# underdoc-wang/STC-GNN

Hardware: NVIDIA B200
Metric: train samples/s (fwd+bwd), SF-shape STC cell stack (higher is better)
Workload: dtype f32

## Files before the change

### stc_gnn_b200/csrc/stc_conv_tc.cu

```cuda
#include "stc_conv_common.cuh"
#include "stc_tc.cuh"

#include <stdlib.h>

namespace stc {

using namespace tc;

struct TcFwdPlan {
  int npt;
  int Dp;
  int KBL;
  int KB;
  int Ntot;
  int Npad;
  int nacc;
  int nmain;
  int tmem_cols;
  int ntiles;
  int x_bulk;
  int PS;
  uint32_t off_a, off_b, off_sh, off_sx, off_se, off_q, off_bias, off_bar, smem_bytes;
};

__device__ __forceinline__ void tc_issue_tile_loads(const ConvArgs& a, const TcFwdPlan& p, int tile, float* stage_h,
                                                    float* stage_x, uint64_t* bar) {
  const long long total_nodes = (long long)a.B * a.N;
  const long long g0 = (long long)tile * p.npt;
  const int nv = (int)min((long long)p.npt, total_nodes - g0);
  const long long R = total_nodes * a.C;
  const int CH = a.C * a.h, CD = a.C * a.Din;
  uint32_t bytes = (uint32_t)(a.Ks * nv * CH * 4);
  if (p.x_bulk) bytes += (uint32_t)(a.Ks * nv * CD * 4);
  mbar_arrive_expect_tx(bar, bytes);
  for (int k = 0; k < a.Ks; ++k) {
    const float* hsrc = (k == 0 ? a.h0 : a.yh + (long long)(k - 1) * R * a.h) + g0 * CH;
    bulk_g2s(stage_h + (size_t)k * 128 * a.h, hsrc, (uint32_t)(nv * CH * 4), bar);
    if (!p.x_bulk) continue;
    float* dst = stage_x + (size_t)k * 128 * a.Din;
    if (k > 0) {
      bulk_g2s(dst, a.yx + (long long)(k - 1) * R * a.Din + g0 * CD, (uint32_t)(nv * CD * 4), bar);
    } else {
      long long g = g0;
      int left = nv;
      while (left > 0) {
        const long long b = g / a.N;
        const int m = (int)(g - b * a.N);
        const int seg = min(left, a.N - m);
        bulk_g2s(dst, a.x0 + b * a.x0_bs + (long long)m * CD, (uint32_t)(seg * CD * 4), bar);
        dst += seg * CD;
        g += seg;
        left -= seg;
      }
    }
  }
}

__device__ __forceinline__ void tc_prefetch_tile(const ConvArgs& a, const TcFwdPlan& p, int tile) {
  const long long total_nodes = (long long)a.B * a.N;
  const long long g0 = (long long)tile * p.npt;
  const int nv = (int)min((long long)p.npt, total_nodes - g0);
  const long long R = total_nodes * a.C;
  const int CH = a.C * a.h, CD = a.C * a.Din;
  const uint32_t hb = (uint32_t)(nv * CH * 4), xb = (uint32_t)(nv * CD * 4);
  for (int k = 0; k < a.Ks; ++k) {
    l2_prefetch((k == 0 ? a.h0 : a.yh + (long long)(k - 1) * R * a.h) + g0 * CH, hb);
    if (!p.x_bulk) continue;
    if (k > 0) {
      l2_prefetch(a.yx + (long long)(k - 1) * R * a.Din + g0 * CD, xb);
    } else {
      long long g = g0;
      int left = nv;
      while (left > 0) {
        const long long b = g / a.N;
        const int m = (int)(g - b * a.N);
        const int seg = min(left, a.N - m);
        l2_prefetch(a.x0 + b * a.x0_bs + (long long)m * CD, (uint32_t)(seg * CD * 4));
        g += seg;
        left -= seg;
      }
    }
  }
  if (a.Hprev != a.h0) l2_prefetch(a.Hprev + g0 * CH, hb);
  if (a.phase != 0) l2_prefetch(a.u + g0 * CH, hb);
}

constexpr int TC_APM = 3;

__device__ __forceinline__ void tc_read_acc8(uint32_t tl, const TcFwdPlan& p, int c0, float (&v)[8]) {
  if (p.nmain == 1) {
    uint32_t t0[8], t1[8];
    tmem_ld8_async(tl + (uint32_t)(p.Npad + c0), t1);
    tmem_ld8_async(tl + (uint32_t)c0, t0);
    tmem_ld_wait();
    tmem_ld_pin8(t0); tmem_ld_pin8(t1);
#pragma unroll
    for (int i = 0; i < 8; ++i) v[i] = __uint_as_float(t1[i]) + __uint_as_float(t0[i]);
    return;
  }
  float t[8];
  tmem_ld8(tl + (uint32_t)(p.nmain * p.Npad + c0), v);
  for (int m = 0; m < p.nmain; ++m) {
    tmem_ld8(tl + (uint32_t)(m * p.Npad + c0), t);
#pragma unroll
    for (int i = 0; i < 8; ++i) v[i] += t[i];
  }
}

template <int NG>
__device__ __forceinline__ void tc_fwd_epilogue_fast(const ConvArgs& a, const TcFwdPlan& p, uint32_t tl, float* Pm,
                                                     const float* Qs, const float* bias_s, const float* stage_e,
                                                     int erow, int enode, int ecat, int half, bool valid,
                                                     long long gr) {
  const int h = a.h, C = a.C, Hout = a.Hout;
  const int cb = half * 8;
  uint32_t sm1[NG][8], mn1[NG][8];
#pragma unroll
  for (int g = 0; g < NG; ++g) {
    tmem_ld8_async(tl + (uint32_t)(p.Npad + Hout + 16 * g + cb), sm1[g]);
    tmem_ld8_async(tl + (uint32_t)(Hout + 16 * g + cb), mn1[g]);
  }
  tmem_ld_wait();
#pragma unroll
  for (int g = 0; g < NG; ++g) {
    tmem_ld_pin8(sm1[g]); tmem_ld_pin8(mn1[g]);
    float t[8];
#pragma unroll
    for (int i = 0; i < 8; ++i) t[i] = __uint_as_float(sm1[g][i]) + __uint_as_float(mn1[g][i]);
    float* pm = Pm + erow * p.PS + 16 * g + cb;
    *reinterpret_cast<float4*>(pm) = make_float4(t[0], t[1], t[2], t[3]);
    *reinterpret_cast<float4*>(pm + 4) = make_float4(t[4], t[5], t[6], t[7]);
    if (a.Psave && valid) {
      float* ps = a.Psave + gr * (long long)Hout + 16 * g + cb;
      *reinterpret_cast<float4*>(ps) = make_float4(t[0], t[1], t[2], t[3]);
      *reinterpret_cast<float4*>(ps + 4) = make_float4(t[4], t[5], t[6], t[7]);
    }
  }
  uint32_t sm0[NG][8], mn0[NG][8];
#pragma unroll
  for (int g = 0; g < NG; ++g) {
    tmem_ld8_async(tl + (uint32_t)(p.Npad + 16 * g + cb), sm0[g]);
    tmem_ld8_async(tl + (uint32_t)(16 * g + cb), mn0[g]);
  }
  __syncthreads();
  tmem_ld_wait();
  float v[NG][8];
#pragma unroll
  for (int g = 0; g < NG; ++g) {
    tmem_ld_pin8(sm0[g]); tmem_ld_pin8(mn0[g]);
#pragma unroll
    for (int i = 0; i < 8; ++i) v[g][i] = __uint_as_float(sm0[g][i]) + __uint_as_float(mn0[g][i]);
  }
  {
    const float* pp = Pm + (enode * C) * p.PS + cb;
#pragma unroll 5
    for (int cp = 0; cp < C; ++cp) {
      const float w = Qs[cp * C + ecat];
#pragma unroll
      for (int g = 0; g < NG; ++g) {
        const float4 x0 = *reinterpret_cast<const float4*>(pp + cp * p.PS + 16 * g);
        const float4 x1 = *reinterpret_cast<const float4*>(pp + cp * p.PS + 16 * g + 4);
        v[g][0] = fmaf(w, x0.x, v[g][0]); v[g][1] = fmaf(w, x0.y, v[g][1]);
        v[g][2] = fmaf(w, x0.z, v[g][2]); v[g][3] = fmaf(w, x0.w, v[g][3]);
        v[g][4] = fmaf(w, x1.x, v[g][4]); v[g][5] = fmaf(w, x1.y, v[g][5]);
        v[g][6] = fmaf(w, x1.z, v[g][6]); v[g][7] = fmaf(w, x1.w, v[g][7]);
      }
    }
  }
  if (!valid) return;
#pragma unroll
  for (int g = 0; g < NG; ++g) {
    const float4 b0 = *reinterpret_cast<const float4*>(bias_s + 16 * g + cb);
    const float4 b1 = *reinterpret_cast<const float4*>(bias_s + 16 * g + cb + 4);
    v[g][0] += b0.x; v[g][1] += b0.y; v[g][2] += b0.z; v[g][3] += b0.w;
    v[g][4] += b1.x; v[g][5] += b1.y; v[g][6] += b1.z; v[g][7] += b1.w;
    if (a.act == STC_ACT_RELU) {
#pragma unroll
      for (int i = 0; i < 8; ++i) v[g][i] = fmaxf(v[g][i], 0.f);
    }
  }
  if (a.phase == 0) {
#pragma unroll
    for (int g = 0; g < NG; ++g) {
#pragma unroll
      for (int i = 0; i < 8; ++i) v[g][i] = sigmoidf_fast(v[g][i]);
      const int col = 16 * g + cb;
      if (col < h) {
        float* dst = a.u + gr * h + col;
        *reinterpret_cast<float4*>(dst) = make_float4(v[g][0], v[g][1], v[g][2], v[g][3]);
        *reinterpret_cast<float4*>(dst + 4) = make_float4(v[g][4], v[g][5], v[g][6], v[g][7]);
      } else {
        const int ch = col - h;
        const float4 h0 = *reinterpret_cast<const float4*>(stage_e + erow * h + ch);
        const float4 h1 = *reinterpret_cast<const float4*>(stage_e + erow * h + ch + 4);
        float* dr = a.r + gr * h + ch;
        *reinterpret_cast<float4*>(dr) = make_float4(v[g][0], v[g][1], v[g][2], v[g][3]);
        *reinterpret_cast<float4*>(dr + 4) = make_float4(v[g][4], v[g][5], v[g][6], v[g][7]);
        float* drh = a.rH + gr * h + ch;
        *reinterpret_cast<float4*>(drh) = make_float4(v[g][0] * h0.x, v[g][1] * h0.y, v[g][2] * h0.z, v[g][3] * h0.w);
        *reinterpret_cast<float4*>(drh + 4) = make_float4(v[g][4] * h1.x, v[g][5] * h1.y, v[g][6] * h1.z, v[g][7] * h1.w);
      }
    }
  } else {
#pragma unroll
    for (int g = 0; g < NG; ++g) {
      const int col = 16 * g + cb;
      const long long o = gr * h + col;
      float cc[8], hn[8];
      const float4 u0 = *reinterpret_cast<const float4*>(stage_e + 128 * h + erow * h + col);
      const float4 u1 = *reinterpret_cast<const float4*>(stage_e + 128 * h + erow * h + col + 4);
      const float4 p0 = *reinterpret_cast<const float4*>(stage_e + erow * h + col);
      const float4 p1 = *reinterpret_cast<const float4*>(stage_e + erow * h + col + 4);
      const float uu[8] = {u0.x, u0.y, u0.z, u0.w, u1.x, u1.y, u1.z, u1.w};
      const float hp[8] = {p0.x, p0.y, p0.z, p0.w, p1.x, p1.y, p1.z, p1.w};
#pragma unroll
      for (int i = 0; i < 8; ++i) {
        cc[i] = tanhf_fast(v[g][i]);
        hn[i] = fmaf(uu[i], cc[i] - hp[i], hp[i]);
      }
      *reinterpret_cast<float4*>(a.c + o) = make_float4(cc[0], cc[1], cc[2], cc[3]);
      *reinterpret_cast<float4*>(a.c + o + 4) = make_float4(cc[4], cc[5], cc[6], cc[7]);
      *reinterpret_cast<float4*>(a.Hnew + o) = make_float4(hn[0], hn[1], hn[2], hn[3]);
      *reinterpret_cast<float4*>(a.Hnew + o + 4) = make_float4(hn[4], hn[5], hn[6], hn[7]);
    }
  }
}

template <int NG>
__global__ void __launch_bounds__(CV_THREADS, 2)
tc_conv_fwd_kernel(const ConvArgs a, const TcFwdPlan p) {
  extern __shared__ __align__(1024) uint8_t smem[];
  if ((smem_u32(smem) & 1023u) != 0u) __trap();
  const int tid = threadIdx.x, warp = tid >> 5, lane = tid & 31;
  const int C = a.C, L = a.Din + a.h, h = a.h, Din = a.Din, Hout = a.Hout;
  const uint32_t atomA = 128 * ATOM_ROW_BYTES;
  const uint32_t atomB = (uint32_t)p.Npad * ATOM_ROW_BYTES;
  uint8_t* A_hi = smem + p.off_a;
  uint8_t* A_lo = A_hi + atomA;
  float* Pm = reinterpret_cast<float*>(A_hi);
  uint8_t* B_hi = smem + p.off_b;
  uint8_t* B_lo = B_hi + (size_t)p.nacc * atomB;
  float* stage_h = reinterpret_cast<float*>(smem + p.off_sh);
  float* stage_x = reinterpret_cast<float*>(smem + p.off_sx);
  float* Qs = reinterpret_cast<float*>(smem + p.off_q);
  float* bias_s = reinterpret_cast<float*>(smem + p.off_bias);
  float* stage_e = reinterpret_cast<float*>(smem + p.off_se);
  uint64_t* mma_bar = reinterpret_cast<uint64_t*>(smem + p.off_bar);
  uint64_t* load_bar = mma_bar + 1;
  uint64_t* epi_bar = mma_bar + 2;
  uint32_t* tmem_slot = reinterpret_cast<uint32_t*>(mma_bar + 3);

  if (tid == 0) {
    mbar_init(mma_bar, 1);
    mbar_init(load_bar, 1);
    mbar_init(epi_bar, 1);
    mbar_fence_init();
  }
  if (warp == 0) tmem_alloc(tmem_slot, (uint32_t)p.tmem_cols);
  for (int i = tid; i < (a.Kc - 1) * C * C; i += CV_THREADS) Qs[i] = a.Q[C * C + i];
  for (int i = tid; i < Hout; i += CV_THREADS) bias_s[i] = a.bias ? a.bias[i] : 0.f;
  for (int i = tid; i < a.Ks * 128 * h; i += CV_THREADS) stage_h[i] = 0.f;
  for (int i = tid; i < a.Ks * 128 * Din; i += CV_THREADS) stage_x[i] = 0.f;
  for (int k = 0; k < a.Ks; ++k)
    for (int j = 0; j < p.KB; ++j) {
      uint8_t* bh = B_hi + (size_t)(k * p.KB + j) * atomB;
      uint8_t* bl = B_lo + (size_t)(k * p.KB + j) * atomB;
      for (int it = tid; it < p.Npad * 8; it += CV_THREADS) {
        const int n = it >> 3, qq = it & 7;
        const int c = n / Hout, o = n - c * Hout;
        float v[4];
#pragma unroll
        for (int i = 0; i < 4; ++i) {
          const int kb = j * ATOM_K + qq * 4 + i;
          const int l = kb < h ? Din + kb : (kb - h < Din ? kb - h : -1);
          v[i] = (n < p.Ntot && l >= 0) ? a.W[((size_t)(k * a.Kc + c) * L + l) * Hout + o] : 0.f;
        }
        store_split4(bh, bl, atom_chunk_offset(n, qq), make_float4(v[0], v[1], v[2], v[3]));
      }
    }
  fence_async_smem();
  fence_before_sync();
  __syncthreads();
  fence_after_sync();
  const int warp_u = uniform_warp_index();
  const uint32_t tmem_base = uniform_u32(*tmem_slot);
  const uint32_t idesc = make_idesc_tf32(128, p.Npad);
  const uint32_t d_small = tmem_base + (uint32_t)(p.nmain * p.Npad);
  const long long total_nodes = (long long)a.B * a.N;
  const long long R = total_nodes * C;
  const uint64_t dA_hi = make_smem_desc_sw128(smem_u32(A_hi)), dA_lo = make_smem_desc_sw128(smem_u32(A_lo));
  const uint64_t dB_hi = make_smem_desc_sw128(smem_u32(B_hi)), dB_lo = make_smem_desc_sw128(smem_u32(B_lo));

  const int q = tid & 7, r0 = tid >> 3;
  uint32_t aoff[4];
#pragma unroll
  for (int i = 0; i < 4; ++i) aoff[i] = atom_chunk_offset(r0 + 32 * i, q);
  const int lane_base = (warp & 3) * 32, half = warp >> 2;
  const int erow = lane_base + lane;
  const int enode = erow / C, ecat = erow - enode * C;
  const uint32_t tl = tmem_base + ((uint32_t)lane_base << 16);

  uint32_t mma_phase = 0, load_phase = 0, epi_phase = 0;
  bool mma_pending = false;
  const bool tracing = a.trace != nullptr && blockIdx.x == 0 && tid == 0;
  int trace_it = 0;
  if (warp_u == 1 && elect_one_sync() && (int)blockIdx.x < p.ntiles) tc_issue_tile_loads(a, p, blockIdx.x, stage_h, stage_x, load_bar);

  for (int tile = blockIdx.x; tile < p.ntiles; tile += gridDim.x) {
    const long long g0 = (long long)tile * p.npt;
    const int nodes_valid = (int)min((long long)p.npt, total_nodes - g0);
    const int rows_valid = nodes_valid * C;
    STC_TRACE(0);
    if (warp_u == 1 && elect_one_sync()) {
      const uint32_t eb = (uint32_t)(rows_valid * h * 4);
      mbar_arrive_expect_tx(epi_bar, a.phase == 0 ? eb : 2 * eb);
      bulk_g2s(stage_e, a.Hprev + g0 * C * h, eb, epi_bar);
      if (a.phase != 0) bulk_g2s(stage_e + 128 * h, a.u + g0 * C * h, eb, epi_bar);
      if ((a.opt & OPT_L2_PREFETCH) && tile + (int)gridDim.x < p.ntiles) tc_prefetch_tile(a, p, tile + gridDim.x);
    }
    mbar_wait(load_bar, load_phase);
    load_phase ^= 1u;
    if (!p.x_bulk) {
      for (int k = 0; k < a.Ks; ++k) {
        float* dst = stage_x + (size_t)k * 128 * Din;
        const int per_node = C * Din;
        for (int idx = tid; idx < nodes_valid * per_node; idx += CV_THREADS) {
          const int node = idx / per_node, rem = idx - node * per_node;
          const long long g = g0 + node;
          const float* src;
          if (k == 0) {
            const long long b = g / a.N;
            src = a.x0 + b * a.x0_bs + (g - b * a.N) * per_node;
          } else {
            src = a.yx + (long long)(k - 1) * R * Din + g * per_node;
          }
          dst[idx] = src[rem];
        }
      }
      __syncthreads();
    }
    STC_TRACE(1);
    bool acc_small = false;
    int ai = 0;
    for (int k = 0; k < a.Ks; ++k) {
      const float* sh = stage_h + (size_t)k * 128 * h;
      const float* sx = stage_x + (size_t)k * 128 * Din;
      for (int j = 0; j < p.KB; ++j, ++ai) {
        const int kb = j * ATOM_K + q * 4;
        const bool from_h = kb < h;
        float4 vv[4];
        if (from_h || (p.x_bulk && kb - h < Din)) {
          const float* bp = from_h ? sh + kb : sx + (kb - h);
          const int st = from_h ? h : Din;
#pragma unroll
          for (int i = 0; i < 4; ++i) vv[i] = *reinterpret_cast<const float4*>(bp + (r0 + 32 * i) * st);
        } else {
          const int xi = kb - h;
#pragma unroll
          for (int i = 0; i < 4; ++i) {
            float e[4] = {0.f, 0.f, 0.f, 0.f};
            const float* sp = sx + (r0 + 32 * i) * Din + xi;
#pragma unroll
            for (int t = 0; t < 4; ++t)
              if (xi + t < Din) e[t] = sp[t];
            vv[i] = make_float4(e[0], e[1], e[2], e[3]);
          }
        }
        float4 vh[4], vl[4];
#pragma unroll
        for (int i = 0; i < 4; ++i) {
          split_tf32(vv[i].x, vh[i].x, vl[i].x); split_tf32(vv[i].y, vh[i].y, vl[i].y);
          split_tf32(vv[i].z, vh[i].z, vl[i].z); split_tf32(vv[i].w, vh[i].w, vl[i].w);
        }
        if (mma_pending) {
          mbar_wait(mma_bar, mma_phase);
          mma_phase ^= 1u;
          mma_pending = false;
          if (ai == p.nacc - 1) STC_TRACE(3);
        }
#pragma unroll
        for (int i = 0; i < 4; ++i) {
          *reinterpret_cast<float4*>(A_hi + aoff[i]) = vh[i];
          *reinterpret_cast<float4*>(A_lo + aoff[i]) = vl[i];
        }
        if (ai == 0) STC_TRACE(12);
        fence_async_smem();
        if (ai == 0) STC_TRACE(13);
        __syncthreads();
        if (ai == 0) STC_TRACE(2);
        if (warp_u == 1 && ai == p.nacc - 1 && tile + (int)gridDim.x < p.ntiles && elect_one_sync())
          tc_issue_tile_loads(a, p, tile + gridDim.x, stage_h, stage_x, load_bar);
        if (warp_u == 0 && elect_one_sync()) {
          fence_after_sync();
          const int kleft = p.KBL - j * ATOM_K;
          const int ksteps = kleft >= ATOM_K ? 4 : (kleft + 7) / 8;
          const uint64_t bo = (uint64_t)(((uint32_t)ai * atomB) >> 4);
          const uint32_t d_main = tmem_base + (uint32_t)((ai / TC_APM) * p.Npad);
          uint32_t acc_main = (ai % TC_APM) != 0 ? 1u : 0u;
#pragma unroll 4
          for (int ks = 0; ks < ksteps; ++ks) {
            const uint64_t ko = (uint64_t)(ks * 2);
            mma_tf32(d_small, dA_lo + ko, dB_hi + bo + ko, idesc, acc_small ? 1u : 0u);
            mma_tf32(d_small, dA_hi + ko, dB_lo + bo + ko, idesc, 1u);
            mma_tf32(d_main, dA_hi + ko, dB_hi + bo + ko, idesc, acc_main);
            acc_main = 1u;
            acc_small = true;
          }
          if (ai == 0) STC_TRACE(8);
          if (ai == p.nacc - 1) STC_TRACE(10);
          mma_commit(mma_bar);
          if (ai == 0) STC_TRACE(9);
          if (ai == p.nacc - 1) STC_TRACE(11);
        }
        acc_small = true;
        mma_pending = true;
      }
    }
    STC_TRACE(4);
    mbar_wait(mma_bar, mma_phase);
    mma_phase ^= 1u;
    mma_pending = false;
    fence_after_sync();
    STC_TRACE(5);
    mbar_wait(epi_bar, epi_phase);
    epi_phase ^= 1u;
    STC_TRACE(6);
    const bool valid = erow < rows_valid;
    const long long gr = g0 * C + erow;
    if constexpr (NG != 0) {
      tc_fwd_epilogue_fast<NG>(a, p, tl, Pm, Qs, bias_s, stage_e, erow, enode, ecat, half, valid, gr);
    } else {
      for (int c0 = half * 8; c0 < Hout; c0 += 16) {
        float v[8];
        tc_read_acc8(tl, p, c0, v);
        for (int c = 1; c < a.Kc; ++c) {
          float t[8];
          tc_read_acc8(tl, p, c * Hout + c0, t);
          __syncthreads();
          *reinterpret_cast<float4*>(Pm + erow * p.PS + c0) = make_float4(t[0], t[1], t[2], t[3]);
          *reinterpret_cast<float4*>(Pm + erow * p.PS + c0 + 4) = make_float4(t[4], t[5], t[6], t[7]);
          if (a.Psave && valid) {
            float4* ps = reinterpret_cast<float4*>(a.Psave + gr * (long long)((a.Kc - 1) * Hout) + (c - 1) * Hout + c0);
            ps[0] = make_float4(t[0], t[1], t[2], t[3]);
            ps[1] = make_float4(t[4], t[5], t[6], t[7]);
          }
          __syncthreads();
          const float* Qc = Qs + (size_t)(c - 1) * C * C;
          const float* pp = Pm + (enode * C) * p.PS + c0;
          for (int cp = 0; cp < C; ++cp) {
            const float w = Qc[cp * C + ecat];
            const float4 x0 = *reinterpret_cast<const float4*>(pp + cp * p.PS);
            const float4 x1 = *reinterpret_cast<const float4*>(pp + cp * p.PS + 4);
            v[0] = fmaf(w, x0.x, v[0]); v[1] = fmaf(w, x0.y, v[1]); v[2] = fmaf(w, x0.z, v[2]); v[3] = fmaf(w, x0.w, v[3]);
            v[4] = fmaf(w, x1.x, v[4]); v[5] = fmaf(w, x1.y, v[5]); v[6] = fmaf(w, x1.z, v[6]); v[7] = fmaf(w, x1.w, v[7]);
          }
        }
        if (!valid) continue;
#pragma unroll
        for (int i = 0; i < 8; ++i) {
          float pre = v[i] + bias_s[c0 + i];
          if (a.act == STC_ACT_RELU) pre = fmaxf(pre, 0.f);
          v[i] = pre;
        }
        if (a.phase == 0) {
#pragma unroll
          for (int i = 0; i < 8; ++i) v[i] = sigmoidf_fast(v[i]);
          if (c0 < h) {
            float4* dst = reinterpret_cast<float4*>(a.u + gr * h + c0);
            dst[0] = make_float4(v[0], v[1], v[2], v[3]);
            dst[1] = make_float4(v[4], v[5], v[6], v[7]);
          } else {
            const long long o = gr * h + (c0 - h);
            const float4 h0 = *reinterpret_cast<const float4*>(stage_e + erow * h + (c0 - h));
            const float4 h1 = *reinterpret_cast<const float4*>(stage_e + erow * h + (c0 - h) + 4);
            float4* dr = reinterpret_cast<float4*>(a.r + o);
            dr[0] = make_float4(v[0], v[1], v[2], v[3]);
            dr[1] = make_float4(v[4], v[5], v[6], v[7]);
            float4* drh = reinterpret_cast<float4*>(a.rH + o);
            drh[0] = make_float4(v[0] * h0.x, v[1] * h0.y, v[2] * h0.z, v[3] * h0.w);
            drh[1] = make_float4(v[4] * h1.x, v[5] * h1.y, v[6] * h1.z, v[7] * h1.w);
          }
        } else {
          const long long o = gr * h + c0;
          float uu[8], hp[8], cc[8], hn[8];
          *reinterpret_cast<float4*>(uu) = *reinterpret_cast<const float4*>(stage_e + 128 * h + erow * h + c0);
          *reinterpret_cast<float4*>(uu + 4) = *reinterpret_cast<const float4*>(stage_e + 128 * h + erow * h + c0 + 4);
          *reinterpret_cast<float4*>(hp) = *reinterpret_cast<const float4*>(stage_e + erow * h + c0);
          *reinterpret_cast<float4*>(hp + 4) = *reinterpret_cast<const float4*>(stage_e + erow * h + c0 + 4);
#pragma unroll
          for (int i = 0; i < 8; ++i) {
            cc[i] = tanhf_fast(v[i]);
            hn[i] = fmaf(uu[i], cc[i] - hp[i], hp[i]);
          }
          float4* dc = reinterpret_cast<float4*>(a.c + o);
          dc[0] = make_float4(cc[0], cc[1], cc[2], cc[3]);
          dc[1] = make_float4(cc[4], cc[5], cc[6], cc[7]);
          float4* dh = reinterpret_cast<float4*>(a.Hnew + o);
          dh[0] = make_float4(hn[0], hn[1], hn[2], hn[3]);
          dh[1] = make_float4(hn[4], hn[5], hn[6], hn[7]);
        }
      }
    }
    STC_TRACE(7);
    ++trace_it;
    fence_before_sync();
    fence_async_smem();
    __syncthreads();
  }
  __syncthreads();
  if (warp == 0) tmem_dealloc(tmem_base, (uint32_t)p.tmem_cols);
}

template <int NG>
__device__ __forceinline__ void tc_fwd_epilogue_regs(const ConvArgs& a, const TcFwdPlan& p, uint32_t tl, float* Pm,
                                                     const float* Qs, const float* bias_s, const float4 (&hp)[2],
                                                     const float4 (&uu)[2], int erow, int enode, int ecat, int half,
                                                     bool valid, long long gr) {
  const int h = a.h, C = a.C, Hout = a.Hout;
  const int cb = half * 8;
  uint32_t sm1[NG][8], mn1[NG][8];
#pragma unroll
  for (int g = 0; g < NG; ++g) {
    tmem_ld8_async(tl + (uint32_t)(p.Npad + Hout + 16 * g + cb), sm1[g]);
    tmem_ld8_async(tl + (uint32_t)(Hout + 16 * g + cb), mn1[g]);
  }
  tmem_ld_wait();
#pragma unroll
  for (int g = 0; g < NG; ++g) {
    tmem_ld_pin8(sm1[g]); tmem_ld_pin8(mn1[g]);
    float t[8];
#pragma unroll
    for (int i = 0; i < 8; ++i) t[i] = __uint_as_float(sm1[g][i]) + __uint_as_float(mn1[g][i]);
    float* pm = Pm + erow * p.PS + 16 * g + cb;
    *reinterpret_cast<float4*>(pm) = make_float4(t[0], t[1], t[2], t[3]);
    *reinterpret_cast<float4*>(pm + 4) = make_float4(t[4], t[5], t[6], t[7]);
    if (a.Psave && valid) {
      float* ps = a.Psave + gr * (long long)Hout + 16 * g + cb;
      *reinterpret_cast<float4*>(ps) = make_float4(t[0], t[1], t[2], t[3]);
      *reinterpret_cast<float4*>(ps + 4) = make_float4(t[4], t[5], t[6], t[7]);
    }
  }
  uint32_t sm0[NG][8], mn0[NG][8];
#pragma unroll
  for (int g = 0; g < NG; ++g) {
    tmem_ld8_async(tl + (uint32_t)(p.Npad + 16 * g + cb), sm0[g]);
    tmem_ld8_async(tl + (uint32_t)(16 * g + cb), mn0[g]);
  }
  __syncthreads();
  tmem_ld_wait();
  float v[NG][8];
#pragma unroll
  for (int g = 0; g < NG; ++g) {
    tmem_ld_pin8(sm0[g]); tmem_ld_pin8(mn0[g]);
#pragma unroll
    for (int i = 0; i < 8; ++i) v[g][i] = __uint_as_float(sm0[g][i]) + __uint_as_float(mn0[g][i]);
  }
  {
    const float* pp = Pm + (enode * C) * p.PS + cb;
#pragma unroll 5
    for (int cp = 0; cp < C; ++cp) {
      const float w = Qs[cp * C + ecat];
#pragma unroll
      for (int g = 0; g < NG; ++g) {
        const float4 x0 = *reinterpret_cast<const float4*>(pp + cp * p.PS + 16 * g);
        const float4 x1 = *reinterpret_cast<const float4*>(pp + cp * p.PS + 16 * g + 4);
        v[g][0] = fmaf(w, x0.x, v[g][0]); v[g][1] = fmaf(w, x0.y, v[g][1]);
        v[g][2] = fmaf(w, x0.z, v[g][2]); v[g][3] = fmaf(w, x0.w, v[g][3]);
        v[g][4] = fmaf(w, x1.x, v[g][4]); v[g][5] = fmaf(w, x1.y, v[g][5]);
        v[g][6] = fmaf(w, x1.z, v[g][6]); v[g][7] = fmaf(w, x1.w, v[g][7]);
      }
    }
  }
  if (!valid) return;
#pragma unroll
  for (int g = 0; g < NG; ++g) {
    const float4 b0 = *reinterpret_cast<const float4*>(bias_s + 16 * g + cb);
    const float4 b1 = *reinterpret_cast<const float4*>(bias_s + 16 * g + cb + 4);
    v[g][0] += b0.x; v[g][1] += b0.y; v[g][2] += b0.z; v[g][3] += b0.w;
    v[g][4] += b1.x; v[g][5] += b1.y; v[g][6] += b1.z; v[g][7] += b1.w;
    if (a.act == STC_ACT_RELU) {
#pragma unroll
      for (int i = 0; i < 8; ++i) v[g][i] = fmaxf(v[g][i], 0.f);
    }
  }
  const float hpv[8] = {hp[0].x, hp[0].y, hp[0].z, hp[0].w, hp[1].x, hp[1].y, hp[1].z, hp[1].w};
  if (a.phase == 0) {
#pragma unroll
    for (int g = 0; g < NG; ++g) {
#pragma unroll
      for (int i = 0; i < 8; ++i) v[g][i] = sigmoidf_fast(v[g][i]);
      const int col = 16 * g + cb;
      if (col < h) {
        float* dst = a.u + gr * h + col;
        *reinterpret_cast<float4*>(dst) = make_float4(v[g][0], v[g][1], v[g][2], v[g][3]);
        *reinterpret_cast<float4*>(dst + 4) = make_float4(v[g][4], v[g][5], v[g][6], v[g][7]);
      } else {
        const int ch = col - h;
        float* dr = a.r + gr * h + ch;
        *reinterpret_cast<float4*>(dr) = make_float4(v[g][0], v[g][1], v[g][2], v[g][3]);
        *reinterpret_cast<float4*>(dr + 4) = make_float4(v[g][4], v[g][5], v[g][6], v[g][7]);
        float* drh = a.rH + gr * h + ch;
        *reinterpret_cast<float4*>(drh) = make_float4(v[g][0] * hpv[0], v[g][1] * hpv[1], v[g][2] * hpv[2], v[g][3] * hpv[3]);
        *reinterpret_cast<float4*>(drh + 4) = make_float4(v[g][4] * hpv[4], v[g][5] * hpv[5], v[g][6] * hpv[6], v[g][7] * hpv[7]);
      }
    }
  } else {
    const float uuv[8] = {uu[0].x, uu[0].y, uu[0].z, uu[0].w, uu[1].x, uu[1].y, uu[1].z, uu[1].w};
    const long long o = gr * h + cb;
    float cc[8], hn[8];
#pragma unroll
    for (int i = 0; i < 8; ++i) {
      cc[i] = tanhf_fast(v[0][i]);
      hn[i] = fmaf(uuv[i], cc[i] - hpv[i], hpv[i]);
    }
    *reinterpret_cast<float4*>(a.c + o) = make_float4(cc[0], cc[1], cc[2], cc[3]);
    *reinterpret_cast<float4*>(a.c + o + 4) = make_float4(cc[4], cc[5], cc[6], cc[7]);
    *reinterpret_cast<float4*>(a.Hnew + o) = make_float4(hn[0], hn[1], hn[2], hn[3]);
    *reinterpret_cast<float4*>(a.Hnew + o + 4) = make_float4(hn[4], hn[5], hn[6], hn[7]);
  }
}

template <int NG>
__global__ void __launch_bounds__(CV_THREADS, 2)
tc_conv_fwd_at_kernel(const ConvArgs a, const TcFwdPlan p) {
  extern __shared__ __align__(1024) uint8_t smem[];
  if ((smem_u32(smem) & 1023u) != 0u) __trap();
  const int tid = threadIdx.x, warp = tid >> 5, lane = tid & 31;
  const int C = a.C, L = a.Din + a.h, Din = a.Din, Hout = a.Hout;
  constexpr int h = 16;
  const uint32_t atomB = (uint32_t)p.Npad * ATOM_ROW_BYTES;
  float* Pm = reinterpret_cast<float*>(smem + p.off_a);
  uint8_t* B_hi = smem + p.off_b;
  uint8_t* B_lo = B_hi + atomB;
  float* Qs = reinterpret_cast<float*>(smem + p.off_q);
  float* bias_s = reinterpret_cast<float*>(smem + p.off_bias);
  uint64_t* mma_bar = reinterpret_cast<uint64_t*>(smem + p.off_bar);
  uint32_t* tmem_slot = reinterpret_cast<uint32_t*>(mma_bar + 1);

  if (tid == 0) {
    mbar_init(mma_bar, 1);
    mbar_fence_init();
  }
  if (warp == 0) tmem_alloc(tmem_slot, (uint32_t)p.tmem_cols);
  for (int i = tid; i < C * C; i += CV_THREADS) Qs[i] = a.Q[C * C + i];
  for (int i = tid; i < Hout; i += CV_THREADS) bias_s[i] = a.bias ? a.bias[i] : 0.f;
  for (int k = 0; k < 2; ++k) {
    uint8_t* bh = B_hi + (size_t)k * 2 * atomB;
    uint8_t* bl = B_lo + (size_t)k * 2 * atomB;
    for (int it = tid; it < p.Npad * 8; it += CV_THREADS) {
      const int n = it >> 3, qq = it & 7;
      const int c = n / Hout, o = n - c * Hout;
      float v[4];
#pragma unroll
      for (int i = 0; i < 4; ++i) {
        const int kb = qq * 4 + i;
        const int l = kb < h ? Din + kb : (kb - h < Din ? kb - h : -1);
        v[i] = (n < p.Ntot && l >= 0) ? a.W[((size_t)(k * 2 + c) * L + l) * Hout + o] : 0.f;
      }
      store_split4(bh, bl, atom_chunk_offset(n, qq), make_float4(v[0], v[1], v[2], v[3]));
    }
  }
  fence_async_smem();
  fence_before_sync();
  __syncthreads();
  fence_after_sync();
  const int warp_u = uniform_warp_index();
  const uint32_t tmem_base = uniform_u32(*tmem_slot);
  const uint32_t idesc = make_idesc_tf32(128, p.Npad), idesc2 = make_idesc_tf32(128, 2 * p.Npad);
  const uint32_t d_main = tmem_base, d_small = tmem_base + (uint32_t)p.Npad;
  const uint32_t colA = (uint32_t)(2 * p.Npad);
  const uint64_t dB_hi = make_smem_desc_sw128(smem_u32(B_hi));
  const int ksteps = p.KBL >> 3;
  const long long total_nodes = (long long)a.B * a.N;
  const long long R = total_nodes * C;

  const int sp = warp & 3, half = warp >> 2;
  const int erow = sp * 32 + lane;
  const int enode = erow / C, ecat = erow - enode * C;
  const uint32_t tl = tmem_base + ((uint32_t)(sp * 32) << 16);
  const uint32_t tA = tl + colA + (uint32_t)(half * 32);
  const bool xvec = p.x_bulk != 0;
  uint32_t mma_phase = 0;
  const bool tracing = a.trace != nullptr && blockIdx.x == 0 && tid == 0;
  int trace_it = 0;
  for (int tile = blockIdx.x; tile < p.ntiles; tile += gridDim.x) {
    const long long g0 = (long long)tile * p.npt;
    const int nodes_valid = (int)min((long long)p.npt, total_nodes - g0);
    const int rows_valid = nodes_valid * C;
    const bool valid = erow < rows_valid;
    const long long gr = g0 * C + erow;
    STC_TRACE(0);
    if ((a.opt & OPT_L2_PREFETCH) && warp_u == 1 && tile + (int)gridDim.x < p.ntiles && elect_one_sync())
      tc_prefetch_tile(a, p, tile + gridDim.x);
    float4 xv[8];
#pragma unroll
    for (int i = 0; i < 8; ++i) xv[i] = make_float4(0.f, 0.f, 0.f, 0.f);
    if (valid) {
      const float* hs = (half == 0 ? a.h0 : a.yh) + gr * h;
#pragma unroll
      for (int i = 0; i < 4; ++i) xv[i] = *reinterpret_cast<const float4*>(hs + 4 * i);
      const float* xs;
      if (half == 0) {
        const long long g = g0 + enode;
        const long long b = g / a.N;
        xs = a.x0 + b * a.x0_bs + ((g - b * a.N) * C + ecat) * Din;
      } else {
        xs = a.yx + gr * Din;
      }
      if (xvec) {
#pragma unroll
        for (int i = 0; i < 4; ++i)
          if (4 * i < Din) xv[4 + i] = *reinterpret_cast<const float4*>(xs + 4 * i);
      } else {
        float e[16];
#pragma unroll
        for (int i = 0; i < 16; ++i) e[i] = i < Din ? xs[i] : 0.f;
#pragma unroll
        for (int i = 0; i < 4; ++i) xv[4 + i] = make_float4(e[4 * i], e[4 * i + 1], e[4 * i + 2], e[4 * i + 3]);
      }
    }
    STC_TRACE(1);
#pragma unroll
    for (int i = 0; i < 4; ++i) {
      float hi[8], lo[8];
      split_tf32(xv[2 * i].x, hi[0], lo[0]); split_tf32(xv[2 * i].y, hi[1], lo[1]);
      split_tf32(xv[2 * i].z, hi[2], lo[2]); split_tf32(xv[2 * i].w, hi[3], lo[3]);
      split_tf32(xv[2 * i + 1].x, hi[4], lo[4]); split_tf32(xv[2 * i + 1].y, hi[5], lo[5]);
      split_tf32(xv[2 * i + 1].z, hi[6], lo[6]); split_tf32(xv[2 * i + 1].w, hi[7], lo[7]);
      tmem_st8(tA + (uint32_t)(8 * i), hi);
      tmem_st8(tA + 64u + (uint32_t)(8 * i), lo);
    }
    tmem_st_wait();
    STC_TRACE(12);
    fence_before_sync();
    STC_TRACE(13);
    __syncthreads();
    STC_TRACE(2);
    STC_TRACE(3);
    if (warp_u == 0 && elect_one_sync()) {
      fence_after_sync();
      uint32_t acc = 0u;
#pragma unroll
      for (int ai = 0; ai < 2; ++ai) {
        const uint64_t bo = (uint64_t)(((uint32_t)ai * 2u * atomB) >> 4);
        for (int ks = 0; ks < ksteps; ++ks) {
          const uint64_t ko = (uint64_t)(ks * 2);
          const uint32_t ah = tmem_base + colA + (uint32_t)(ai * 32 + ks * 8), al = ah + 64u;
          mma_tf32_atmem(d_main, ah, dB_hi + bo + ko, idesc2, acc);
          mma_tf32_atmem(d_small, al, dB_hi + bo + ko, idesc, 1u);
          acc = 1u;
        }
      }
      STC_TRACE(8);
      STC_TRACE(10);
      mma_commit(mma_bar);
      STC_TRACE(9);
      STC_TRACE(11);
    }
    float4 hp[2], uu[2];
    hp[0] = hp[1] = uu[0] = uu[1] = make_float4(0.f, 0.f, 0.f, 0.f);
    if (valid) {
      const float* hsrc = a.Hprev + gr * h + half * 8;
      hp[0] = *reinterpret_cast<const float4*>(hsrc);
      hp[1] = *reinterpret_cast<const float4*>(hsrc + 4);
      if (a.phase != 0) {
        const float* usrc = a.u + gr * h + half * 8;
        uu[0] = *reinterpret_cast<const float4*>(usrc);
        uu[1] = *reinterpret_cast<const float4*>(usrc + 4);
      }
    }
    STC_TRACE(4);
    mbar_wait(mma_bar, mma_phase);
    mma_phase ^= 1u;
    fence_after_sync();
    STC_TRACE(5);
    STC_TRACE(6);
    tc_fwd_epilogue_regs<NG>(a, p, tl, Pm, Qs, bias_s, hp, uu, erow, enode, ecat, half, valid, gr);
    STC_TRACE(7);
    ++trace_it;
    fence_before_sync();
    __syncthreads();
  }
  __syncthreads();
  if (warp == 0) tmem_dealloc(tmem_base, (uint32_t)p.tmem_cols);
}

static bool tc_disabled() {
  static int cached = -1;
  if (cached < 0) {
    const char* e = getenv("STC_DISABLE_TC");
    cached = (e && e[0] && e[0] != '0') ? 1 : 0;
  }
  return cached == 1;
}

static bool aligned16p(const void* p) { return (reinterpret_cast<uintptr_t>(p) & 15) == 0; }

bool conv_tc_eligible(const ConvArgs& a) {
  if (tc_disabled()) return false;
  if (a.h % 8 != 0 || a.Hout % 16 != 0 || a.C > 128) return false;
  const int Dp = (a.Din + 7) & ~7, KBL = a.h + Dp, KB = (KBL + ATOM_K - 1) / ATOM_K;
  const int Nf = (a.Kc * a.Hout + 15) & ~15;
  if (Nf > 256 || (a.Ks * KB + 1) * Nf > 512) return false;
  if ((size_t)128 * (a.Hout + 4) * sizeof(float) > 2 * 128 * ATOM_ROW_BYTES) return false;
  const size_t fwd_smem = 2 * 128 * ATOM_ROW_BYTES + 2 * (size_t)a.Ks * KB * Nf * ATOM_ROW_BYTES +
                          (size_t)a.Ks * 128 * (a.h + a.Din) * sizeof(float) + (size_t)2 * 128 * a.h * sizeof(float) +
                          (size_t)a.Kc * a.C * a.C * sizeof(float) + 64;
  if (fwd_smem > 200 * 1024) return false;
  const int Nb = (a.Ks * KBL + 15) & ~15, KA = (a.Kc * a.Hout + ATOM_K - 1) / ATOM_K;
  if (Nb > 256 || (KA + 1) * Nb > 512) return false;
  const size_t dx_smem = 2 * 128 * ATOM_ROW_BYTES + 2 * (size_t)KA * Nb * ATOM_ROW_BYTES +
                         (size_t)128 * (a.Hout + 4 + a.h + (a.Kc - 1) * a.Hout) * sizeof(float) +
                         (size_t)2 * a.Kc * a.C * a.C * sizeof(float) + 256;
  if (dx_smem > 200 * 1024) return false;
  return true;
}

int try_launch_conv_fwd_tc(const ConvArgs& a, cudaStream_t st, bool* handled) {
  *handled = false;
  if (!conv_tc_eligible(a)) return STC_OK;
  const int L = a.Din + a.h, P = a.Ks * a.Kc;
  if (!aligned16p(a.u) || !aligned16p(a.Hprev) || !aligned16p(a.r) || !aligned16p(a.rH) || !aligned16p(a.c) ||
      !aligned16p(a.Hnew) || !aligned16p(a.h0) || !aligned16p(a.yh) || !aligned16p(a.Psave)) {
    set_error("tcgen05 path needs 16-byte aligned state / workspace tensors");
    return STC_ERR_BAD_ARG;
  }
  auto declined = [&](const char* why) {
    set_error("tcgen05 forward declined an eligible shape (%s): N=%d C=%d Din=%d h=%d Ks=%d Kc=%d Hout=%d", why, a.N, a.C,
              a.Din, a.h, a.Ks, a.Kc, a.Hout);
    return STC_ERR_UNSUPPORTED;
  };
  TcFwdPlan p;
  p.npt = 128 / a.C;
  p.Dp = (a.Din + 7) & ~7;
  p.KBL = a.h + p.Dp;
  p.KB = (p.KBL + ATOM_K - 1) / ATOM_K;
  p.Ntot = a.Kc * a.Hout;
  p.Npad = (p.Ntot + 15) & ~15;
  if (p.Npad > 256) return declined("N tile");
  p.nacc = a.Ks * p.KB;
  p.nmain = (p.nacc + TC_APM - 1) / TC_APM;
  p.tmem_cols = 32;
  while (p.tmem_cols < (p.nmain + 1) * p.Npad) p.tmem_cols *= 2;
  if (p.tmem_cols > 512) return declined("tensor memory columns");
  p.PS = a.Hout + 4;
  if ((size_t)128 * p.PS * sizeof(float) > 2 * 128 * ATOM_ROW_BYTES) return declined("exchange buffer");
  p.x_bulk = (a.Din % 4 == 0) && (a.x0_bs % 4 == 0) && aligned16p(a.x0) && aligned16p(a.yx);
  const long long total_nodes = (long long)a.B * a.N;
  p.ntiles = ceil_div(total_nodes, p.npt);
  const size_t atomB = (size_t)p.Npad * ATOM_ROW_BYTES;
  size_t o = 0;
  p.off_a = (uint32_t)o; o += 2 * 128 * ATOM_ROW_BYTES;
  p.off_b = (uint32_t)o; o += 2 * (size_t)p.nacc * atomB;
  p.off_sh = (uint32_t)o; o += (size_t)a.Ks * 128 * a.h * sizeof(float);
  p.off_sx = (uint32_t)o; o += round_up((size_t)a.Ks * 128 * a.Din * sizeof(float), 16);
  p.off_se = (uint32_t)o; o += (size_t)2 * 128 * a.h * sizeof(float);
  p.off_q = (uint32_t)o; o += (size_t)(a.Kc > 1 ? a.Kc - 1 : 0) * a.C * a.C * sizeof(float);
  o = round_up(o, 16);
  p.off_bias = (uint32_t)o; o += (size_t)a.Hout * sizeof(float);
  o = round_up(o, 16);
  p.off_bar = (uint32_t)o; o += 48;
  p.smem_bytes = (uint32_t)o;
  const bool smem_over = p.smem_bytes > 200 * 1024;
  int ng = 0;
  if (a.Kc == 2 && p.nmain == 1 && (a.Hout == 16 || a.Hout == 32) && !(a.opt & OPT_GENERIC_EPILOGUE)) ng = a.Hout / 16;
  auto kern = ng == 2 ? tc_conv_fwd_kernel<2> : (ng == 1 ? tc_conv_fwd_kernel<1> : tc_conv_fwd_kernel<0>);
  const bool at = ng != 0 && a.Ks == 2 && a.h == 16 && p.KB == 1 && !(a.opt & OPT_SMEM_A);
  if (at) {
    kern = ng == 2 ? tc_conv_fwd_at_kernel<2> : tc_conv_fwd_at_kernel<1>;
    size_t q = 0;
    p.off_a = (uint32_t)q; q += round_up((size_t)128 * p.PS * sizeof(float), 1024);
    p.off_b = (uint32_t)q; q += 2 * (size_t)2 * atomB;
    p.off_q = (uint32_t)q; q += round_up((size_t)a.C * a.C * sizeof(float), 16);
    p.off_bias = (uint32_t)q; q += round_up((size_t)a.Hout * sizeof(float), 16);
    p.off_bar = (uint32_t)q; q += 32;
    p.smem_bytes = (uint32_t)q;
    p.tmem_cols = 256;
  }
  if (!at && smem_over) return declined("shared memory");
  STC_TRY(set_smem(kern, p.smem_bytes));
  int ctas_per_sm = (int)((228 * 1024) / (p.smem_bytes + 1024));
  if (ctas_per_sm < 1) ctas_per_sm = 1;
  if (ctas_per_sm > 2) ctas_per_sm = 2;
  if (ctas_per_sm * p.tmem_cols > 512) ctas_per_sm = 512 / p.tmem_cols;
  int grid = device_sm_count() * ctas_per_sm;
  if (grid > p.ntiles) grid = p.ntiles;
  const double R = (double)total_nodes * a.C;
  ScopedKernelTimer _t(KK_TC_CONV_FWD, st,
                       4.0 * R * (a.Ks * L + (a.phase == 0 ? 3 * a.h : 4 * a.h)) + 4.0 * P * L * a.Hout);
  kern<<<grid, CV_THREADS, p.smem_bytes, st>>>(a, p);
  STC_LAUNCH_OK("tc_conv_fwd_kernel");
  *handled = true;
  return STC_OK;
}

__global__ void __launch_bounds__(CV_THREADS, 1)
tf32x3_gemm_kernel(const float* __restrict__ A, const float* __restrict__ Bm, float* __restrict__ D, int M, int N,
                   int K, int Npad, int tmem_cols, int mode, int nmain, int small) {
  extern __shared__ __align__(1024) uint8_t smem[];
  if ((smem_u32(smem) & 1023u) != 0u) __trap();
  const int tid = threadIdx.x, warp = tid >> 5, lane = tid & 31;
  const uint32_t atomA = 128 * ATOM_ROW_BYTES, atomB = (uint32_t)Npad * ATOM_ROW_BYTES;
  uint8_t* A_hi = smem;
  uint8_t* A_lo = A_hi + atomA;
  uint8_t* B_hi = A_lo + atomA;
  uint8_t* B_lo = B_hi + atomB;
  uint64_t* bar = reinterpret_cast<uint64_t*>(B_lo + atomB);
  uint32_t* tmem_slot = reinterpret_cast<uint32_t*>(bar + 1);
  if (tid == 0) {
    mbar_init(bar, 1);
    mbar_fence_init();
  }
  if (warp == 0) tmem_alloc(tmem_slot, (uint32_t)tmem_cols);
  fence_before_sync();
  __syncthreads();
  fence_after_sync();
  const uint32_t tmem_base = *tmem_slot;
  const uint32_t idesc = make_idesc_tf32(128, Npad);
  const int m0 = blockIdx.x * 128;
  uint32_t phase = 0;
  bool acc_main[16], acc_small = false;
  for (int i = 0; i < 16; ++i) acc_main[i] = false;
  const int natoms = (K + ATOM_K - 1) / ATOM_K;
  for (int j = 0; j < natoms; ++j) {
    if (j > 0) {
      mbar_wait(bar, phase);
      phase ^= 1u;
    }
    for (int it = tid; it < 128 * 8; it += CV_THREADS) {
      const int row = it >> 3, q = it & 7;
      float v[4], hi[4], lo[4];
#pragma unroll
      for (int i = 0; i < 4; ++i) {
        const int k = j * ATOM_K + q * 4 + i;
        v[i] = (m0 + row < M && k < K) ? A[(size_t)(m0 + row) * K + k] : 0.f;
        if (mode & 1) split_tf32_trunc(v[i], hi[i], lo[i]); else split_tf32(v[i], hi[i], lo[i]);
      }
      const uint32_t off = atom_chunk_offset(row, q);
      *reinterpret_cast<float4*>(A_hi + off) = make_float4(hi[0], hi[1], hi[2], hi[3]);
      *reinterpret_cast<float4*>(A_lo + off) = make_float4(lo[0], lo[1], lo[2], lo[3]);
    }
    for (int it = tid; it < Npad * 8; it += CV_THREADS) {
      const int n = it >> 3, q = it & 7;
      float v[4], hi[4], lo[4];
#pragma unroll
      for (int i = 0; i < 4; ++i) {
        const int k = j * ATOM_K + q * 4 + i;
        v[i] = (n < N && k < K) ? Bm[(size_t)k * N + n] : 0.f;
        if (mode & 1) split_tf32_trunc(v[i], hi[i], lo[i]); else split_tf32(v[i], hi[i], lo[i]);
      }
      const uint32_t off = atom_chunk_offset(n, q);
      *reinterpret_cast<float4*>(B_hi + off) = make_float4(hi[0], hi[1], hi[2], hi[3]);
      *reinterpret_cast<float4*>(B_lo + off) = make_float4(lo[0], lo[1], lo[2], lo[3]);
    }
    fence_async_smem();
    __syncthreads();
    if (tid == 0) {
      fence_after_sync();
      const int kleft = K - j * ATOM_K;
      const int ksteps = kleft >= ATOM_K ? 4 : (kleft + 7) / 8;
      const int mi = j % nmain;
      const uint32_t d_main = tmem_base + (uint32_t)(mi * Npad);
      if (small) {
        const uint32_t d_small = tmem_base + (uint32_t)(nmain * Npad);
        mma_atom_3x_split(d_main, d_small, smem_u32(A_hi), smem_u32(A_lo), smem_u32(B_hi), smem_u32(B_lo), ksteps, idesc,
                          acc_main[mi], acc_small);
      } else {
        mma_atom_3x(d_main, smem_u32(A_hi), smem_u32(A_lo), smem_u32(B_hi), smem_u32(B_lo), ksteps, idesc, acc_main[mi]);
      }
      mma_commit(bar);
    }
  }
  mbar_wait(bar, phase);
  fence_after_sync();
  {
    const int lane_base = (warp & 3) * 32, half = warp >> 2;
    const int row = m0 + lane_base + lane;
    const int nchunks = Npad / 8;
    const int nbuf = (natoms < nmain ? natoms : nmain);
    for (int ch = half; ch < nchunks; ch += 2) {
      float acc[8], v[8];
      if (small) {
        tmem_ld8(tmem_base + ((uint32_t)lane_base << 16) + (uint32_t)(nmain * Npad + ch * 8), acc);
      } else {
        for (int i = 0; i < 8; ++i) acc[i] = 0.f;
      }
      for (int b = 0; b < nbuf; ++b) {
        tmem_ld8(tmem_base + ((uint32_t)lane_base << 16) + (uint32_t)(b * Npad + ch * 8), v);
        for (int i = 0; i < 8; ++i) acc[i] += v[i];
      }
      if (row < M)
        for (int i = 0; i < 8; ++i)
          if (ch * 8 + i < N) D[(size_t)row * N + ch * 8 + i] = acc[i];
    }
  }
  fence_before_sync();
  __syncthreads();
  if (warp == 0) tmem_dealloc(tmem_base, (uint32_t)tmem_cols);
}

struct MnLayout {
  int variant;
  uint32_t colblk;
  uint32_t kgroup;
  __device__ __forceinline__ uint32_t off(int k, int ch) const {
    if (variant == 2) return (uint32_t)(k >> 3) * kgroup + (uint32_t)ch * 128u + (uint32_t)(k & 7) * 16u;
    return (uint32_t)(ch >> 3) * colblk + mn32_chunk_offset(k, ch & 7);
  }
  __device__ __forceinline__ uint64_t desc(uint32_t base, int ks) const {
    if (variant == 2) {
      uint64_t d = 0;
      d |= (uint64_t)(((base + ks * kgroup) >> 4) & 0x3FFF);
      d |= (uint64_t)((kgroup >> 4) & 0x3FFF) << 16;
      d |= (uint64_t)((128u >> 4) & 0x3FFF) << 32;
      d |= (uint64_t)1 << 46;
      return d;
    }
    const uint32_t a = base + ks * 2 * MN32_GROUP_BYTES;
    return variant == 0 ? make_smem_desc_mn32(a, colblk, MN32_GROUP_BYTES) : make_smem_desc_mn32(a, MN32_GROUP_BYTES, colblk);
  }
};

__global__ void __launch_bounds__(CV_THREADS, 1)
tf32x3_gemm_mn_kernel(const float* __restrict__ A, const float* __restrict__ Bm, float* __restrict__ D, int M, int N,
                      int K, int Npad, int tmem_cols, int variant) {
  extern __shared__ __align__(1024) uint8_t smem[];
  if ((smem_u32(smem) & 1023u) != 0u) __trap();
  const int tid = threadIdx.x, warp = tid >> 5, lane = tid & 31;
  const int ncolB = (Npad + 31) / 32;
  const uint32_t colblk = 32 * ATOM_ROW_BYTES;
  const MnLayout la{variant, colblk, 32u * 128u};
  const MnLayout lb{variant, colblk, (uint32_t)(ncolB * 8) * 128u};
  uint8_t* A_hi = smem;
  uint8_t* A_lo = A_hi + 4 * colblk;
  uint8_t* B_hi = A_lo + 4 * colblk;
  uint8_t* B_lo = B_hi + ncolB * colblk;
  uint64_t* bar = reinterpret_cast<uint64_t*>(B_lo + ncolB * colblk);
  uint32_t* tmem_slot = reinterpret_cast<uint32_t*>(bar + 1);
  if (tid == 0) {
    mbar_init(bar, 1);
    mbar_fence_init();
  }
  if (warp == 0) tmem_alloc(tmem_slot, (uint32_t)tmem_cols);
  fence_before_sync();
  __syncthreads();
  fence_after_sync();
  const uint32_t tmem_base = *tmem_slot;
  const uint32_t idesc = make_idesc_tf32_mn(128, Npad);
  const int m0 = blockIdx.x * 128;
  uint32_t phase = 0;
  const int nchunksK = (K + 31) / 32;
  bool acc_main = false, acc_small = false;
  for (int j = 0; j < nchunksK; ++j) {
    if (j > 0) {
      mbar_wait(bar, phase);
      phase ^= 1u;
    }
    for (int it = tid; it < 32 * 32; it += CV_THREADS) {
      const int k = it >> 5, ch = it & 31;
      float v[4];
#pragma unroll
      for (int i = 0; i < 4; ++i) {
        const int m = ch * 4 + i, kk = j * 32 + k;
        v[i] = (m0 + m < M && kk < K) ? A[(size_t)(m0 + m) * K + kk] : 0.f;
      }
      store_split4(A_hi, A_lo, la.off(k, ch), make_float4(v[0], v[1], v[2], v[3]));
    }
    for (int it = tid; it < 32 * ncolB * 8; it += CV_THREADS) {
      const int k = it / (ncolB * 8), ch = it - k * (ncolB * 8);
      float v[4];
#pragma unroll
      for (int i = 0; i < 4; ++i) {
        const int n = ch * 4 + i, kk = j * 32 + k;
        v[i] = (n < N && kk < K) ? Bm[(size_t)kk * N + n] : 0.f;
      }
      store_split4(B_hi, B_lo, lb.off(k, ch), make_float4(v[0], v[1], v[2], v[3]));
    }
    fence_async_smem();
    __syncthreads();
    if (tid == 0) {
      fence_after_sync();
      const int kleft = K - j * 32;
      const int ksteps = kleft >= 32 ? 4 : (kleft + 7) / 8;
      for (int ks = 0; ks < ksteps; ++ks) {
        const uint64_t ah = la.desc(smem_u32(A_hi), ks), al = la.desc(smem_u32(A_lo), ks);
        const uint64_t bh = lb.desc(smem_u32(B_hi), ks), bl = lb.desc(smem_u32(B_lo), ks);
        mma_tf32(tmem_base + (uint32_t)Npad, al, bh, idesc, acc_small ? 1u : 0u);
        mma_tf32(tmem_base + (uint32_t)Npad, ah, bl, idesc, 1u);
        mma_tf32(tmem_base, ah, bh, idesc, acc_main ? 1u : 0u);
        acc_main = acc_small = true;
      }
      mma_commit(bar);
    }
  }
  mbar_wait(bar, phase);
  fence_after_sync();
  {
    const int lane_base = (warp & 3) * 32, half = warp >> 2;
    const int row = m0 + lane_base + lane;
    for (int ch = half; ch < Npad / 8; ch += 2) {
      float v[8], t[8];
      tmem_ld8(tmem_base + ((uint32_t)lane_base << 16) + (uint32_t)(Npad + ch * 8), v);
      tmem_ld8(tmem_base + ((uint32_t)lane_base << 16) + (uint32_t)(ch * 8), t);
      if (row < M)
        for (int i = 0; i < 8; ++i)
          if (ch * 8 + i < N) D[(size_t)row * N + ch * 8 + i] = v[i] + t[i];
    }
  }
  fence_before_sync();
  __syncthreads();
  if (warp == 0) tmem_dealloc(tmem_base, (uint32_t)tmem_cols);
}

int launch_tf32x3_gemm(const float* A, const float* Bm, float* D, int M, int N, int K, cudaStream_t st) {
  if (M <= 0 || N <= 0 || K <= 0 || N > 256) {
    set_error("tf32x3 gemm self-test: need M,K > 0 and 0 < N <= 256");
    return STC_ERR_BAD_ARG;
  }
  int mode = 0, nmain = 1, small = 0;
  if (const char* e = getenv("STC_TC_TEST_MODE")) mode = atoi(e);
  if (const char* e = getenv("STC_TC_TEST_NMAIN")) nmain = atoi(e);
  if (const char* e = getenv("STC_TC_TEST_SMALL")) small = atoi(e);
  const int Npad = (N + 15) & ~15;
  if (mode & 2) {
    int cols = 32;
    while (cols < 2 * Npad) cols *= 2;
    const size_t smem_mn = (size_t)(8 + 2 * ((Npad + 31) / 32)) * 32 * ATOM_ROW_BYTES + 64;
    STC_TRY(set_smem(tf32x3_gemm_mn_kernel, smem_mn));
    ScopedKernelTimer _t(KK_TC_GEMM_TEST, st, 4.0 * ((double)M * K + (double)K * N + (double)M * N));
    int variant = 0;
    if (const char* e = getenv("STC_TC_MN_VARIANT")) variant = atoi(e);
    tf32x3_gemm_mn_kernel<<<ceil_div(M, 128), CV_THREADS, smem_mn, st>>>(A, Bm, D, M, N, K, Npad, cols, variant);
    STC_LAUNCH_OK("tf32x3_gemm_mn_kernel");
    return STC_OK;
  }
  if (nmain < 1) nmain = 1;
  if (nmain > 15) nmain = 15;
  while ((nmain + (small ? 1 : 0)) * Npad > 512 && nmain > 1) --nmain;
  int tmem_cols = 32;
  while (tmem_cols < (nmain + (small ? 1 : 0)) * Npad) tmem_cols *= 2;
  const size_t smem = 2 * 128 * ATOM_ROW_BYTES + 2 * (size_t)Npad * ATOM_ROW_BYTES + 64;
  STC_TRY(set_smem(tf32x3_gemm_kernel, smem));
  ScopedKernelTimer _t(KK_TC_GEMM_TEST, st, 4.0 * ((double)M * K + (double)K * N + (double)M * N));
  tf32x3_gemm_kernel<<<ceil_div(M, 128), CV_THREADS, smem, st>>>(A, Bm, D, M, N, K, Npad, tmem_cols, mode, nmain, small);
  STC_LAUNCH_OK("tf32x3_gemm_kernel");
  return STC_OK;
}

}
```

### stc_gnn_b200/csrc/stc_conv_tc_bwd.cu

```cuda
#include "stc_conv_common.cuh"
#include "stc_tc.cuh"

namespace stc {

using namespace tc;

constexpr int DX_APM = 3;

struct TcDxPlan {
  int npt, Dp, KBL;
  int N1;
  int Npad;
  int Kdd;
  int KA;
  int nmain;
  int tmem_cols, ntiles;
  int DP;
  int PW;
  int x_vec;
  uint32_t off_a, off_b, off_ds, off_dh, off_ps, off_q, off_acc, off_bar, smem_bytes;
};

struct DxIn {
  float4 dhn, uu, cc, hp, rr, drh;
};
__device__ __forceinline__ void dx_load(const ConvArgs& a, long long o, DxIn& in) {
  in.dhn = *reinterpret_cast<const float4*>(a.dHn + o);
  in.uu = *reinterpret_cast<const float4*>(a.u + o);
  in.cc = *reinterpret_cast<const float4*>(a.c + o);
  if (a.phase == 0) {
    in.hp = *reinterpret_cast<const float4*>(a.Hprev + o);
    in.rr = *reinterpret_cast<const float4*>(a.r + o);
    in.drh = *reinterpret_cast<const float4*>(a.drH + o);
  }
}
__device__ __forceinline__ void dx_adjoint(const ConvArgs& a, const DxIn& in, float4& g0v, float4& g1v, float4& dir) {
  const float4 dhn = in.dhn, uu = in.uu, cc = in.cc;
  if (a.phase == 1) {
    g0v = make_float4(dhn.x * uu.x * (1.f - cc.x * cc.x), dhn.y * uu.y * (1.f - cc.y * cc.y),
                      dhn.z * uu.z * (1.f - cc.z * cc.z), dhn.w * uu.w * (1.f - cc.w * cc.w));
    if (a.act == STC_ACT_RELU) {
      if (!(cc.x > 0.f)) g0v.x = 0.f;
      if (!(cc.y > 0.f)) g0v.y = 0.f;
      if (!(cc.z > 0.f)) g0v.z = 0.f;
      if (!(cc.w > 0.f)) g0v.w = 0.f;
    }
  } else {
    const float4 hp = in.hp, rr = in.rr, drh = in.drh;
    g0v = make_float4(dhn.x * (cc.x - hp.x) * uu.x * (1.f - uu.x), dhn.y * (cc.y - hp.y) * uu.y * (1.f - uu.y),
                      dhn.z * (cc.z - hp.z) * uu.z * (1.f - uu.z), dhn.w * (cc.w - hp.w) * uu.w * (1.f - uu.w));
    g1v = make_float4(drh.x * hp.x * rr.x * (1.f - rr.x), drh.y * hp.y * rr.y * (1.f - rr.y),
                      drh.z * hp.z * rr.z * (1.f - rr.z), drh.w * hp.w * rr.w * (1.f - rr.w));
    if (a.act == STC_ACT_RELU) {
      if (!(uu.x > 0.5f)) g0v.x = 0.f;
      if (!(uu.y > 0.5f)) g0v.y = 0.f;
      if (!(uu.z > 0.5f)) g0v.z = 0.f;
      if (!(uu.w > 0.5f)) g0v.w = 0.f;
      if (!(rr.x > 0.5f)) g1v.x = 0.f;
      if (!(rr.y > 0.5f)) g1v.y = 0.f;
      if (!(rr.z > 0.5f)) g1v.z = 0.f;
      if (!(rr.w > 0.5f)) g1v.w = 0.f;
    }
    dir = make_float4(dhn.x * (1.f - uu.x) + drh.x * rr.x, dhn.y * (1.f - uu.y) + drh.y * rr.y,
                      dhn.z * (1.f - uu.z) + drh.z * rr.z, dhn.w * (1.f - uu.w) + drh.w * rr.w);
  }
}

__device__ __forceinline__ void dx_prefetch_tile(const ConvArgs& a, const TcDxPlan& p, int tile, bool want_dQ) {
  const long long total_nodes = (long long)a.B * a.N;
  const long long g0 = (long long)tile * p.npt;
  const int nv = (int)min((long long)p.npt, total_nodes - g0);
  const long long row0 = g0 * a.C;
  const uint32_t hb = (uint32_t)(nv * a.C * a.h * 4);
  l2_prefetch(a.dHn + row0 * a.h, hb);
  l2_prefetch(a.u + row0 * a.h, hb);
  l2_prefetch(a.c + row0 * a.h, hb);
  if (a.phase == 0) {
    l2_prefetch(a.Hprev + row0 * a.h, hb);
    l2_prefetch(a.r + row0 * a.h, hb);
    l2_prefetch(a.drH + row0 * a.h, hb);
  }
  if (want_dQ) l2_prefetch(a.Psave + row0 * p.PW, (uint32_t)(nv * a.C * p.PW * 4));
  if (a.accum_x && p.x_vec) {
    const uint32_t xb = (uint32_t)(nv * a.C * a.Din * 4);
    const long long R = total_nodes * a.C;
    if (a.dYx0) l2_prefetch(a.dYx0 + row0 * a.Din, xb);
    if (a.dYx)
      for (int k = 1; k < a.Ks; ++k) l2_prefetch(a.dYx + (size_t)(k - 1) * R * a.Din + row0 * a.Din, xb);
  }
}

template <bool FAST, bool AT>
__global__ void __launch_bounds__(CV_THREADS, 2)
tc_conv_bwd_dx_kernel(const ConvArgs a, const TcDxPlan p) {
  extern __shared__ __align__(1024) uint8_t smem[];
  if ((smem_u32(smem) & 1023u) != 0u) __trap();
  const int tid = threadIdx.x, warp = tid >> 5, lane = tid & 31;
  const int C = a.C, L = a.Din + a.h, h = a.h, Din = a.Din, Hout = a.Hout, DP = p.DP;
  const bool want_dQ = a.dQ != nullptr && a.Kc > 1;
  const uint32_t atomA = 128 * ATOM_ROW_BYTES;
  const uint32_t atomB = (uint32_t)p.Npad * ATOM_ROW_BYTES;
  uint8_t* A_hi = smem + p.off_a;
  uint8_t* A_lo = A_hi + atomA;
  uint8_t* B_hi = smem + p.off_b;
  uint8_t* B_lo = B_hi + (AT ? (size_t)atomB : (size_t)p.KA * atomB);
  const size_t bstride = AT ? 2 * (size_t)atomB : (size_t)atomB;
  float* Dsm = reinterpret_cast<float*>(smem + p.off_ds);
  float* Dh = reinterpret_cast<float*>(smem + p.off_dh);
  float* Psm = reinterpret_cast<float*>(smem + p.off_ps);
  float* Qs = reinterpret_cast<float*>(smem + p.off_q);
  float* dQacc = reinterpret_cast<float*>(smem + p.off_acc);
  uint64_t* mma_bar = reinterpret_cast<uint64_t*>(smem + p.off_bar);
  uint64_t* load_bar = mma_bar + 1;
  uint32_t* tmem_slot = reinterpret_cast<uint32_t*>(mma_bar + 2);

  if (tid == 0) {
    mbar_init(mma_bar, 1);
    mbar_init(load_bar, 1);
    mbar_fence_init();
  }
  if (warp == 0) tmem_alloc(tmem_slot, (uint32_t)p.tmem_cols);
  for (int i = tid; i < (a.Kc - 1) * C * C; i += CV_THREADS) {
    Qs[i] = a.Q[C * C + i];
    dQacc[i] = 0.f;
  }
  for (int ja = 0; ja < p.KA; ++ja) {
    uint8_t* bh = B_hi + (size_t)ja * bstride;
    uint8_t* bl = B_lo + (size_t)ja * bstride;
    for (int it = tid; it < p.Npad * 8; it += CV_THREADS) {
      const int n = it >> 3, qq = it & 7;
      const int k = n / p.KBL, kb = n - k * p.KBL;
      const int l = kb < h ? Din + kb : (kb - h < Din ? kb - h : -1);
      float v[4];
#pragma unroll
      for (int i = 0; i < 4; ++i) {
        const int kk = ja * ATOM_K + qq * 4 + i;
        const int c = kk / Hout, o = kk - c * Hout;
        v[i] = (n < p.N1 && l >= 0 && kk < p.Kdd) ? a.W[((size_t)(k * a.Kc + c) * L + l) * Hout + o] : 0.f;
      }
      store_split4(bh, bl, atom_chunk_offset(n, qq), make_float4(v[0], v[1], v[2], v[3]));
    }
  }
  fence_async_smem();
  fence_before_sync();
  __syncthreads();
  fence_after_sync();
  const int warp_u = uniform_warp_index();
  const uint32_t tmem_base = uniform_u32(*tmem_slot);
  const uint32_t idesc = make_idesc_tf32(128, p.Npad), idesc2 = make_idesc_tf32(128, 2 * p.Npad);
  const uint32_t d_small = tmem_base + (uint32_t)(p.nmain * p.Npad);
  const uint64_t dA_hi = make_smem_desc_sw128(smem_u32(A_hi)), dA_lo = make_smem_desc_sw128(smem_u32(A_lo));
  const uint64_t dB_hi = make_smem_desc_sw128(smem_u32(B_hi)), dB_lo = make_smem_desc_sw128(smem_u32(B_lo));
  const long long total_nodes = (long long)a.B * a.N;
  const long long R = total_nodes * C;

  const int q = tid & 7, r0 = tid >> 3;
  uint32_t aoff[4];
  int rnode[4], rcat[4];
#pragma unroll
  for (int i = 0; i < 4; ++i) {
    aoff[i] = atom_chunk_offset(r0 + 32 * i, q);
    rnode[i] = (r0 + 32 * i) / C;
    rcat[i] = (r0 + 32 * i) - rnode[i] * C;
  }
  const int lane_base = (warp & 3) * 32, half = warp >> 2;
  const int erow = lane_base + lane;
  const uint32_t tl = tmem_base + ((uint32_t)lane_base << 16);
  const bool db_fast = a.dbias != nullptr && (CV_THREADS % (h >> 2)) == 0;
  float4 dbs0 = make_float4(0.f, 0.f, 0.f, 0.f), dbs1 = dbs0;
  float db_acc = 0.f;
  const int db_groups = CV_THREADS / Hout, db_col = tid % Hout, db_grp = tid / Hout;
  constexpr int DQ_C = 5;
  const int dq_chunks = Hout >> 2;
  const bool dq_fast = want_dQ && a.Kc == 2 && C <= DQ_C && p.npt * dq_chunks <= CV_THREADS;
  const int dq_node = tid / dq_chunks, dq_oc = (tid - dq_node * dq_chunks) << 2;
  float dq[DQ_C * DQ_C];
#pragma unroll
  for (int i = 0; i < DQ_C * DQ_C; ++i) dq[i] = 0.f;
  uint32_t mma_phase = 0, load_phase = 0;
  bool mma_pending = false;
  const bool tracing = a.trace != nullptr && blockIdx.x == 0 && tid == 0;
  int trace_it = 0;

  for (int tile = blockIdx.x; tile < p.ntiles; tile += gridDim.x) {
    const long long g0 = (long long)tile * p.npt;
    const int nodes_valid = (int)min((long long)p.npt, total_nodes - g0);
    const int rows_valid = nodes_valid * C;
    const long long row0 = g0 * C;
    if (warp_u == 1 && elect_one_sync()) {
      if (want_dQ) {
        const uint32_t bytes = (uint32_t)(rows_valid * p.PW * 4);
        mbar_arrive_expect_tx(load_bar, bytes);
        bulk_g2s(Psm, a.Psave + row0 * p.PW, bytes, load_bar);
      }
      if ((a.opt & OPT_L2_PREFETCH) && tile + (int)gridDim.x < p.ntiles) dx_prefetch_tile(a, p, tile + gridDim.x, want_dQ);
    }
    STC_TRACE(0);
    const int cpr = h >> 2;
    auto emit_item = [&](int row, int j, const float4& g0v, const float4& g1v, const float4& dir, bool live) {
      if (live) {
        *reinterpret_cast<float4*>(a.dpre + (row0 + row) * p.Kdd + j) = g0v;
        if (a.phase == 0) *reinterpret_cast<float4*>(a.dpre + (row0 + row) * p.Kdd + h + j) = g1v;
      }
      if (db_fast) {
        dbs0.x += g0v.x; dbs0.y += g0v.y; dbs0.z += g0v.z; dbs0.w += g0v.w;
        dbs1.x += g1v.x; dbs1.y += g1v.y; dbs1.z += g1v.z; dbs1.w += g1v.w;
      }
      *reinterpret_cast<float4*>(Dsm + row * DP + j) = g0v;
      if (a.phase == 0) {
        *reinterpret_cast<float4*>(Dsm + row * DP + h + j) = g1v;
        *reinterpret_cast<float4*>(Dh + row * h + j) = dir;
      }
    };
    for (int it = tid; it < 128 * cpr; it += CV_THREADS) {
      const int row = it / cpr, j = (it - row * cpr) << 2;
      float4 g0v = make_float4(0.f, 0.f, 0.f, 0.f), g1v = g0v, dir = g0v;
      const bool live = row < rows_valid;
      if (live) {
        DxIn in;
        dx_load(a, (row0 + row) * h + j, in);
        dx_adjoint(a, in, g0v, g1v, dir);
      }
      emit_item(row, j, g0v, g1v, dir, live);
    }
    __syncthreads();
    STC_TRACE(1);
    if (a.dbias && !db_fast && tid < db_groups * Hout) {
      float s = 0.f;
      for (int row = db_grp; row < rows_valid; row += db_groups) s += Dsm[row * DP + db_col];
      db_acc += s;
    }
    if constexpr (AT) {
      const int cw = Hout >> 1;
      const int cbase = cw * half;
      const int enode = erow / C, ecat = erow - enode * C;
      const float* qrow = Qs + ecat * C;
      const uint32_t tA = tl + (uint32_t)(2 * p.Npad);
      const bool two = cw == 16;
      float dm[16];
#pragma unroll
      for (int i = 0; i < 16; ++i) dm[i] = 0.f;
      {
        const float* sp = Dsm + (enode * C) * DP + cbase;
#pragma unroll 5
        for (int d = 0; d < C; ++d) {
          const float w = qrow[d];
          const float4 x0 = *reinterpret_cast<const float4*>(sp + d * DP);
          const float4 x1 = *reinterpret_cast<const float4*>(sp + d * DP + 4);
          dm[0] = fmaf(w, x0.x, dm[0]); dm[1] = fmaf(w, x0.y, dm[1]); dm[2] = fmaf(w, x0.z, dm[2]); dm[3] = fmaf(w, x0.w, dm[3]);
          dm[4] = fmaf(w, x1.x, dm[4]); dm[5] = fmaf(w, x1.y, dm[5]); dm[6] = fmaf(w, x1.z, dm[6]); dm[7] = fmaf(w, x1.w, dm[7]);
          if (two) {
            const float4 x2 = *reinterpret_cast<const float4*>(sp + d * DP + 8);
            const float4 x3 = *reinterpret_cast<const float4*>(sp + d * DP + 12);
            dm[8] = fmaf(w, x2.x, dm[8]); dm[9] = fmaf(w, x2.y, dm[9]); dm[10] = fmaf(w, x2.z, dm[10]); dm[11] = fmaf(w, x2.w, dm[11]);
            dm[12] = fmaf(w, x3.x, dm[12]); dm[13] = fmaf(w, x3.y, dm[13]); dm[14] = fmaf(w, x3.z, dm[14]); dm[15] = fmaf(w, x3.w, dm[15]);
          }
        }
      }
      if (erow < rows_valid) {
        float* dp = a.dpre + (row0 + erow) * p.Kdd + Hout + cbase;
        *reinterpret_cast<float4*>(dp) = make_float4(dm[0], dm[1], dm[2], dm[3]);
        *reinterpret_cast<float4*>(dp + 4) = make_float4(dm[4], dm[5], dm[6], dm[7]);
        if (two) {
          *reinterpret_cast<float4*>(dp + 8) = make_float4(dm[8], dm[9], dm[10], dm[11]);
          *reinterpret_cast<float4*>(dp + 12) = make_float4(dm[12], dm[13], dm[14], dm[15]);
        }
      }
#pragma unroll
      for (int part = 0; part < 2; ++part) {
        if (part * 8 < cw) {
          const int col = cbase + part * 8;
          float hi[8], lo[8];
          {
            const float4 x0 = *reinterpret_cast<const float4*>(Dsm + erow * DP + col);
            const float4 x1 = *reinterpret_cast<const float4*>(Dsm + erow * DP + col + 4);
            split_tf32(x0.x, hi[0], lo[0]); split_tf32(x0.y, hi[1], lo[1]); split_tf32(x0.z, hi[2], lo[2]); split_tf32(x0.w, hi[3], lo[3]);
            split_tf32(x1.x, hi[4], lo[4]); split_tf32(x1.y, hi[5], lo[5]); split_tf32(x1.z, hi[6], lo[6]); split_tf32(x1.w, hi[7], lo[7]);
          }
          tmem_st8(tA + (uint32_t)col, hi);
          tmem_st8(tA + 64u + (uint32_t)col, lo);
#pragma unroll
          for (int i = 0; i < 8; ++i) split_tf32(dm[part * 8 + i], hi[i], lo[i]);
          tmem_st8(tA + (uint32_t)(Hout + col), hi);
          tmem_st8(tA + 64u + (uint32_t)(Hout + col), lo);
        }
      }
      tmem_st_wait();
      STC_TRACE(12);
      fence_before_sync();
      STC_TRACE(13);
      __syncthreads();
      STC_TRACE(2);
      if (warp_u == 0 && elect_one_sync()) {
        fence_after_sync();
        const uint32_t a0 = tmem_base + (uint32_t)(2 * p.Npad);
        uint32_t acc = 0u;
        const int nks = p.Kdd >> 3;
        for (int ks = 0; ks < nks; ++ks) {
          const uint64_t bo = (uint64_t)((((uint32_t)(ks >> 2)) * 2u * atomB) >> 4) + (uint64_t)((ks & 3) * 2);
          const uint32_t ah = a0 + (uint32_t)(ks * 8), al = ah + 64u;
          mma_tf32_atmem(tmem_base, ah, dB_hi + bo, idesc2, acc);
          mma_tf32_atmem(d_small, al, dB_hi + bo, idesc, 1u);
          acc = 1u;
        }
        STC_TRACE(8);
        STC_TRACE(10);
        mma_commit(mma_bar);
        STC_TRACE(9);
        STC_TRACE(11);
      }
      mma_pending = true;
    } else {
      bool acc_small = false;
      for (int ja = 0; ja < p.KA; ++ja) {
        const int kk = ja * ATOM_K + q * 4;
        const int c = kk / Hout, o0 = kk - c * Hout;
        float4 vv[4];
  #pragma unroll
        for (int i = 0; i < 4; ++i) {
          float4 v = make_float4(0.f, 0.f, 0.f, 0.f);
          if (kk < p.Kdd) {
            if (c == 0) {
              v = *reinterpret_cast<const float4*>(Dsm + (r0 + 32 * i) * DP + o0);
            } else {
              const float* Qc = Qs + (size_t)(c - 1) * C * C + rcat[i] * C;
              const float* sp = Dsm + rnode[i] * C * DP + o0;
              for (int d = 0; d < C; ++d) {
                const float w = Qc[d];
                const float4 x = *reinterpret_cast<const float4*>(sp + d * DP);
                v.x = fmaf(w, x.x, v.x); v.y = fmaf(w, x.y, v.y); v.z = fmaf(w, x.z, v.z); v.w = fmaf(w, x.w, v.w);
              }
              if (r0 + 32 * i < rows_valid)
                *reinterpret_cast<float4*>(a.dpre + (row0 + r0 + 32 * i) * p.Kdd + kk) = v;
            }
          }
          vv[i] = v;
        }
        if (mma_pending) {
          mbar_wait(mma_bar, mma_phase);
          mma_phase ^= 1u;
          mma_pending = false;
        }
  #pragma unroll
        for (int i = 0; i < 4; ++i) store_split4(A_hi, A_lo, aoff[i], vv[i]);
        if (ja == 0) STC_TRACE(12);
        fence_async_smem();
        if (ja == 0) STC_TRACE(13);
        __syncthreads();
        if (ja == 0) STC_TRACE(2);
        if (warp_u == 0 && elect_one_sync()) {
          fence_after_sync();
          const int kleft = p.Kdd - ja * ATOM_K;
          const int ksteps = kleft >= ATOM_K ? 4 : (kleft + 7) / 8;
          const uint64_t bo = (uint64_t)(((uint32_t)ja * atomB) >> 4);
          const uint32_t d_main = tmem_base + (uint32_t)((ja / DX_APM) * p.Npad);
          uint32_t acc_main = (ja % DX_APM) != 0 ? 1u : 0u;
  #pragma unroll 4
          for (int ks = 0; ks < ksteps; ++ks) {
            const uint64_t ko = (uint64_t)(ks * 2);
            mma_tf32(d_small, dA_lo + ko, dB_hi + bo + ko, idesc, acc_small ? 1u : 0u);
            mma_tf32(d_small, dA_hi + ko, dB_lo + bo + ko, idesc, 1u);
            mma_tf32(d_main, dA_hi + ko, dB_hi + bo + ko, idesc, acc_main);
            acc_main = 1u;
            acc_small = true;
          }
          if (ja == 0) STC_TRACE(8);
          if (ja == p.KA - 1) STC_TRACE(10);
          mma_commit(mma_bar);
          if (ja == 0) STC_TRACE(9);
          if (ja == p.KA - 1) STC_TRACE(11);
        }
        acc_small = true;
        mma_pending = true;
      }
    }
    STC_TRACE(3);
    float4 xprev[4];
#pragma unroll
    for (int i = 0; i < 4; ++i) xprev[i] = make_float4(0.f, 0.f, 0.f, 0.f);
    if constexpr (FAST) {
      if (a.accum_x && p.x_vec && erow < rows_valid) {
        const float* dbase_pf = (half == 0 ? a.dYx0 : a.dYx);
        if (dbase_pf != nullptr) {
          const float* src = dbase_pf + (row0 + erow) * Din;
#pragma unroll
          for (int i = 0; i < 4; ++i)
            if (4 * i < Din) xprev[i] = *reinterpret_cast<const float4*>(src + 4 * i);
        }
      }
    }
    if (want_dQ) {
      mbar_wait(load_bar, load_phase);
      load_phase ^= 1u;
      const int npairs = (a.Kc - 1) * C * C;
      const int groups = CV_THREADS / npairs;
      if (dq_fast) {
        if (dq_node < nodes_valid) {
          float4 pv[DQ_C], dv[DQ_C];
#pragma unroll
          for (int i = 0; i < DQ_C; ++i) {
            const int ci = i < C ? i : 0;
            pv[i] = *reinterpret_cast<const float4*>(Psm + (dq_node * C + ci) * p.PW + dq_oc);
            dv[i] = *reinterpret_cast<const float4*>(Dsm + (dq_node * C + ci) * DP + dq_oc);
          }
#pragma unroll
          for (int cp = 0; cp < DQ_C; ++cp)
#pragma unroll
            for (int d = 0; d < DQ_C; ++d) {
              float s = dq[cp * DQ_C + d];
              s = fmaf(pv[cp].x, dv[d].x, s); s = fmaf(pv[cp].y, dv[d].y, s);
              s = fmaf(pv[cp].z, dv[d].z, s); s = fmaf(pv[cp].w, dv[d].w, s);
              dq[cp * DQ_C + d] = s;
            }
        }
      } else if (groups >= 1) {
        const int pr = tid % npairs, grp = tid / npairs;
        if (grp < groups) {
          const int c = pr / (C * C), rem = pr - c * C * C, cp = rem / C, d = rem - cp * C;
          float s = 0.f;
          for (int node = grp; node < nodes_valid; node += groups) {
            const float* pp = Psm + (node * C + cp) * p.PW + c * Hout;
            const float* dd = Dsm + (node * C + d) * DP;
            for (int o = 0; o < Hout; o += 4) {
              const float4 x = *reinterpret_cast<const float4*>(pp + o);
              const float4 y = *reinterpret_cast<const float4*>(dd + o);
              s = fmaf(x.x, y.x, s); s = fmaf(x.y, y.y, s); s = fmaf(x.z, y.z, s); s = fmaf(x.w, y.w, s);
            }
          }
          atomicAdd(&dQacc[pr], s);
        }
      } else {
        for (int pr = tid; pr < npairs; pr += CV_THREADS) {
          const int c = pr / (C * C), rem = pr - c * C * C, cp = rem / C, d = rem - cp * C;
          float s = 0.f;
          for (int node = 0; node < nodes_valid; ++node) {
            const float* pp = Psm + (node * C + cp) * p.PW + c * Hout;
            const float* dd = Dsm + (node * C + d) * DP;
            for (int o = 0; o < Hout; ++o) s = fmaf(pp[o], dd[o], s);
          }
          dQacc[pr] += s;
        }
      }
    }
    STC_TRACE(4);
    mbar_wait(mma_bar, mma_phase);
    mma_phase ^= 1u;
    mma_pending = false;
    fence_after_sync();
    STC_TRACE(5);
    const bool valid = erow < rows_valid;
    const long long gr = row0 + erow;
    if constexpr (FAST) {
      const int k = half;
      const uint32_t nb = (uint32_t)(k * p.KBL);
      {
        uint32_t sm[16], mn[16];
        tmem_ld16_async(tl + (uint32_t)p.Npad + nb, sm);
        tmem_ld16_async(tl + nb, mn);
        tmem_ld_wait();
        tmem_ld_pin16(sm); tmem_ld_pin16(mn);
        if (valid) {
          float v[16];
#pragma unroll
          for (int i = 0; i < 16; ++i) v[i] = __uint_as_float(sm[i]) + __uint_as_float(mn[i]);
          if (k == 0 && a.phase == 0) {
#pragma unroll
            for (int i = 0; i < 16; i += 4) {
              const float4 d = *reinterpret_cast<const float4*>(Dh + erow * 16 + i);
              v[i] += d.x; v[i + 1] += d.y; v[i + 2] += d.z; v[i + 3] += d.w;
            }
          }
          float* dst = (k == 0 ? a.dYh0 : a.dYh) + gr * 16;
#pragma unroll
          for (int i = 0; i < 16; i += 4) *reinterpret_cast<float4*>(dst + i) = make_float4(v[i], v[i + 1], v[i + 2], v[i + 3]);
        }
      }
      float* dbase = (k == 0 ? a.dYx0 : a.dYx);
      {
        uint32_t sm[16], mn[16];
        if (p.Dp == 16) {
          tmem_ld16_async(tl + (uint32_t)p.Npad + nb + 16u, sm);
          tmem_ld16_async(tl + nb + 16u, mn);
          tmem_ld_wait();
          tmem_ld_pin16(sm); tmem_ld_pin16(mn);
        } else {
          uint32_t s8[8], m8[8];
          tmem_ld8_async(tl + (uint32_t)p.Npad + nb + 16u, s8);
          tmem_ld8_async(tl + nb + 16u, m8);
          tmem_ld_wait();
          tmem_ld_pin8(s8); tmem_ld_pin8(m8);
#pragma unroll
          for (int i = 0; i < 8; ++i) { sm[i] = s8[i]; mn[i] = m8[i]; sm[i + 8] = 0u; mn[i + 8] = 0u; }
        }
        if (valid && dbase != nullptr) {
          float* dst = dbase + gr * Din;
          if (p.x_vec) {
            float4 o[4];
#pragma unroll
            for (int i = 0; i < 4; ++i)
              o[i] = make_float4(__uint_as_float(sm[4 * i]) + __uint_as_float(mn[4 * i]),
                                 __uint_as_float(sm[4 * i + 1]) + __uint_as_float(mn[4 * i + 1]),
                                 __uint_as_float(sm[4 * i + 2]) + __uint_as_float(mn[4 * i + 2]),
                                 __uint_as_float(sm[4 * i + 3]) + __uint_as_float(mn[4 * i + 3]));
            if (a.accum_x) {
#pragma unroll
              for (int i = 0; i < 4; ++i)
                if (4 * i < Din) { o[i].x += xprev[i].x; o[i].y += xprev[i].y; o[i].z += xprev[i].z; o[i].w += xprev[i].w; }
            }
#pragma unroll
            for (int i = 0; i < 4; ++i)
              if (4 * i < Din) *reinterpret_cast<float4*>(dst + 4 * i) = o[i];
          } else {
#pragma unroll
            for (int i = 0; i < 16; ++i)
              if (i < Din) {
                const float vi = __uint_as_float(sm[i]) + __uint_as_float(mn[i]);
                dst[i] = a.accum_x ? dst[i] + vi : vi;
              }
          }
        }
      }
    } else {
      int k = 0, kb = half * 8;
      for (int n0 = half * 8; n0 < p.Npad; n0 += 16, kb += 16) {
        float v[8];
        if (p.nmain == 1) {
          uint32_t t0[8], t1[8];
          tmem_ld8_async(tl + (uint32_t)(p.Npad + n0), t1);
          tmem_ld8_async(tl + (uint32_t)n0, t0);
          tmem_ld_wait();
          tmem_ld_pin8(t0); tmem_ld_pin8(t1);
#pragma unroll
          for (int i = 0; i < 8; ++i) v[i] = __uint_as_float(t1[i]) + __uint_as_float(t0[i]);
        } else {
          float t[8];
          tmem_ld8(tl + (uint32_t)(p.nmain * p.Npad + n0), v);
          for (int m = 0; m < p.nmain; ++m) {
            tmem_ld8(tl + (uint32_t)(m * p.Npad + n0), t);
#pragma unroll
            for (int i = 0; i < 8; ++i) v[i] += t[i];
          }
        }
        while (kb >= p.KBL) { kb -= p.KBL; ++k; }
        if (!valid || n0 >= p.N1) continue;
        if (kb < h) {
          float* dst = (k == 0 ? a.dYh0 : a.dYh + (size_t)(k - 1) * R * h) + gr * h + kb;
          if (k == 0 && a.phase == 0) {
            const float* dp = Dh + erow * h + kb;
#pragma unroll
            for (int i = 0; i < 8; ++i) v[i] += dp[i];
          }
          reinterpret_cast<float4*>(dst)[0] = make_float4(v[0], v[1], v[2], v[3]);
          reinterpret_cast<float4*>(dst)[1] = make_float4(v[4], v[5], v[6], v[7]);
        } else {
          const int xi = kb - h;
          float* dbase = (k == 0 ? a.dYx0 : a.dYx + (size_t)(k - 1) * R * Din);
          if (dbase == nullptr) continue;
          float* dst = dbase + gr * Din + xi;
          if (p.x_vec && xi + 8 <= Din) {
            float4 o0 = make_float4(v[0], v[1], v[2], v[3]), o1 = make_float4(v[4], v[5], v[6], v[7]);
            if (a.accum_x) {
              const float4 p0 = reinterpret_cast<const float4*>(dst)[0], p1 = reinterpret_cast<const float4*>(dst)[1];
              o0.x += p0.x; o0.y += p0.y; o0.z += p0.z; o0.w += p0.w;
              o1.x += p1.x; o1.y += p1.y; o1.z += p1.z; o1.w += p1.w;
            }
            reinterpret_cast<float4*>(dst)[0] = o0;
            reinterpret_cast<float4*>(dst)[1] = o1;
          } else {
#pragma unroll
            for (int i = 0; i < 8; ++i)
              if (xi + i < Din) dst[i] = a.accum_x ? dst[i] + v[i] : v[i];
          }
        }
      }
    }
    STC_TRACE(6);
    fence_before_sync();
    fence_async_smem();
    __syncthreads();
    STC_TRACE(7);
    ++trace_it;
  }
  if (a.dbias && !db_fast && tid < db_groups * Hout) atomicAdd(&a.dbias[db_col], db_acc);
  __syncthreads();
  if (db_fast) {
    for (int i = tid; i < Hout; i += CV_THREADS) Dsm[i] = 0.f;
    __syncthreads();
    const int cprw = h >> 2;
    float v[8] = {dbs0.x, dbs0.y, dbs0.z, dbs0.w, dbs1.x, dbs1.y, dbs1.z, dbs1.w};
    for (int off = cprw; off < 32; off <<= 1) {
#pragma unroll
      for (int i = 0; i < 8; ++i) v[i] += __shfl_xor_sync(0xffffffffu, v[i], off);
    }
    if (lane < cprw || cprw >= 32) {
      const int j = (tid % cprw) << 2;
      atomicAdd(&Dsm[j + 0], v[0]); atomicAdd(&Dsm[j + 1], v[1]); atomicAdd(&Dsm[j + 2], v[2]); atomicAdd(&Dsm[j + 3], v[3]);
      if (a.phase == 0) {
        atomicAdd(&Dsm[h + j + 0], v[4]); atomicAdd(&Dsm[h + j + 1], v[5]);
        atomicAdd(&Dsm[h + j + 2], v[6]); atomicAdd(&Dsm[h + j + 3], v[7]);
      }
    }
    __syncthreads();
    for (int i = tid; i < Hout; i += CV_THREADS) atomicAdd(&a.dbias[i], Dsm[i]);
  }
  if (dq_fast) {
#pragma unroll
    for (int cp = 0; cp < DQ_C; ++cp)
#pragma unroll
      for (int d = 0; d < DQ_C; ++d) {
        float s = dq[cp * DQ_C + d];
#pragma unroll
        for (int off = 16; off >= 1; off >>= 1) s += __shfl_xor_sync(0xffffffffu, s, off);
        if (lane == 0 && cp < C && d < C) atomicAdd(&dQacc[cp * C + d], s);
      }
  }
  __syncthreads();
  if (want_dQ)
    for (int i = tid; i < (a.Kc - 1) * C * C; i += CV_THREADS) atomicAdd(&a.dQ[C * C + i], dQacc[i]);
  if (warp == 0) tmem_dealloc(tmem_base, (uint32_t)p.tmem_cols);
}

static bool aligned16b(const void* p) { return (reinterpret_cast<uintptr_t>(p) & 15) == 0; }

int try_launch_conv_bwd_dx_tc(const ConvArgs& a, cudaStream_t st, bool* handled) {
  *handled = false;
  if (!conv_tc_eligible(a)) return STC_OK;
  if (!aligned16b(a.dHn) || !aligned16b(a.u) || !aligned16b(a.c) || !aligned16b(a.Hprev) || !aligned16b(a.dpre) ||
      !aligned16b(a.dYh0) || !aligned16b(a.dYh) || !aligned16b(a.Psave) || (a.phase == 0 && (!aligned16b(a.r) || !aligned16b(a.drH)))) {
    set_error("tcgen05 backward needs 16-byte aligned gradient / workspace tensors");
    return STC_ERR_BAD_ARG;
  }
  const int L = a.Din + a.h;
  TcDxPlan p;
  p.npt = 128 / a.C;
  p.Dp = (a.Din + 7) & ~7;
  p.KBL = a.h + p.Dp;
  p.N1 = a.Ks * p.KBL;
  p.Npad = (p.N1 + 15) & ~15;
  p.Kdd = a.Kc * a.Hout;
  p.KA = (p.Kdd + ATOM_K - 1) / ATOM_K;
  p.nmain = (p.KA + DX_APM - 1) / DX_APM;
  p.tmem_cols = 32;
  while (p.tmem_cols < (p.nmain + 1) * p.Npad) p.tmem_cols *= 2;
  p.DP = a.Hout + 4;
  p.PW = (a.Kc - 1) * a.Hout;
  p.x_vec = (a.Din % 4 == 0) && aligned16b(a.dYx0) && aligned16b(a.dYx);
  const long long total_nodes = (long long)a.B * a.N;
  p.ntiles = ceil_div(total_nodes, p.npt);
  const size_t atomB = (size_t)p.Npad * ATOM_ROW_BYTES;
  size_t o = 0;
  p.off_a = (uint32_t)o; o += 2 * 128 * ATOM_ROW_BYTES;
  p.off_b = (uint32_t)o; o += 2 * (size_t)p.KA * atomB;
  p.off_ds = (uint32_t)o; o += (size_t)128 * p.DP * sizeof(float);
  p.off_dh = (uint32_t)o; o += (size_t)128 * a.h * sizeof(float);
  p.off_ps = (uint32_t)o; o += round_up((size_t)128 * p.PW * sizeof(float), 16);
  p.off_q = (uint32_t)o; o += round_up((size_t)(a.Kc > 1 ? a.Kc - 1 : 0) * a.C * a.C * sizeof(float), 16);
  p.off_acc = (uint32_t)o; o += round_up((size_t)(a.Kc > 1 ? a.Kc - 1 : 0) * a.C * a.C * sizeof(float), 16);
  p.off_bar = (uint32_t)o; o += 32;
  p.smem_bytes = (uint32_t)o;
  if (p.smem_bytes > 200 * 1024) {
    set_error("tcgen05 backward tile does not fit (%u B) although the forward ran on the tensor-core path", p.smem_bytes);
    return STC_ERR_UNSUPPORTED;
  }
  const bool fast = a.Ks == 2 && a.h == 16 && a.Din <= 16 && p.nmain == 1 && !(a.opt & OPT_GENERIC_EPILOGUE);
  const bool at = fast && a.Kc == 2 && p.Kdd <= 64 && (a.Hout == 16 || a.Hout == 32) && !(a.opt & OPT_SMEM_A);
  auto kern = at ? tc_conv_bwd_dx_kernel<true, true>
                 : (fast ? tc_conv_bwd_dx_kernel<true, false> : tc_conv_bwd_dx_kernel<false, false>);
  if (at) p.tmem_cols = 256;
  STC_TRY(set_smem(kern, p.smem_bytes));
  int ctas_per_sm = (int)((228 * 1024) / (p.smem_bytes + 1024));
  if (ctas_per_sm < 1) ctas_per_sm = 1;
  if (ctas_per_sm > 2) ctas_per_sm = 2;
  if (ctas_per_sm * p.tmem_cols > 512) ctas_per_sm = 512 / p.tmem_cols;
  int grid = device_sm_count() * ctas_per_sm;
  if (grid > p.ntiles) grid = p.ntiles;
  const double R = (double)total_nodes * a.C;
  ScopedKernelTimer _t(KK_TC_CONV_BWD_DX, st,
                       4.0 * R * ((a.phase == 0 ? 6 * a.h + a.Ks * a.Din : 3 * a.h) + a.Hout + a.Ks * L +
                                  ((a.dQ && a.Kc > 1) ? p.PW : 0)) + 4.0 * a.Ks * a.Kc * L * a.Hout);
  kern<<<grid, CV_THREADS, p.smem_bytes, st>>>(a, p);
  STC_LAUNCH_OK("tc_conv_bwd_dx_kernel");
  *handled = true;
  return STC_OK;
}

}
```

Measured before the change: 61780.

## Warp-specialize tcgen05 conv fwd and bwd-dx kernels with TMA stage ring

Replaces the fast-path forward and backward-dx tensor-core conv kernels with warp-specialized persistent kernels. A producer warp fills a multi-stage TMA ring, converter warps split inputs into TF32 hi/lo in TMEM, an MMA warp issues tcgen05 ops into double-buffered TMEM accumulators, and epilogue warps drain them. Phases are coordinated by mbarrier full/empty pairs. The aim is to overlap loads, conversion, MMA and epilogue across tiles instead of serializing them with __syncthreads. In exchange the kernels run one CTA per SM, allocate all 512 TMEM columns, use more shared memory and much more complex synchronization.

```diff
diff --git a/stc_gnn_b200/csrc/stc_conv_tc.cu b/stc_gnn_b200/csrc/stc_conv_tc.cu
--- a/stc_gnn_b200/csrc/stc_conv_tc.cu
+++ b/stc_gnn_b200/csrc/stc_conv_tc.cu
@@ -20,11 +20,13 @@
   int ntiles;
   int x_bulk;
   int PS;
+  int nst;
   uint32_t off_a, off_b, off_sh, off_sx, off_se, off_q, off_bias, off_bar, smem_bytes;
+  uint32_t stage_bytes;
 };
 
 __device__ __forceinline__ void tc_issue_tile_loads(const ConvArgs& a, const TcFwdPlan& p, int tile, float* stage_h,
-                                                    float* stage_x, uint64_t* bar) {
+                                                    float* stage_x, float* stage_e, uint64_t* bar) {
   const long long total_nodes = (long long)a.B * a.N;
   const long long g0 = (long long)tile * p.npt;
   const int nv = (int)min((long long)p.npt, total_nodes - g0);
@@ -32,7 +34,12 @@
   const int CH = a.C * a.h, CD = a.C * a.Din;
   uint32_t bytes = (uint32_t)(a.Ks * nv * CH * 4);
   if (p.x_bulk) bytes += (uint32_t)(a.Ks * nv * CD * 4);
+  if (stage_e) bytes += (uint32_t)((a.phase == 0 ? 1 : 2) * nv * CH * 4);
   mbar_arrive_expect_tx(bar, bytes);
+  if (stage_e) {
+    bulk_g2s(stage_e, a.Hprev + g0 * CH, (uint32_t)(nv * CH * 4), bar);
+    if (a.phase != 0) bulk_g2s(stage_e + 128 * a.h, a.u + g0 * CH, (uint32_t)(nv * CH * 4), bar);
+  }
   for (int k = 0; k < a.Ks; ++k) {
     const float* hsrc = (k == 0 ? a.h0 : a.yh + (long long)(k - 1) * R * a.h) + g0 * CH;
     bulk_g2s(stage_h + (size_t)k * 128 * a.h, hsrc, (uint32_t)(nv * CH * 4), bar);
@@ -304,7 +311,7 @@
   bool mma_pending = false;
   const bool tracing = a.trace != nullptr && blockIdx.x == 0 && tid == 0;
   int trace_it = 0;
-  if (warp_u == 1 && elect_one_sync() && (int)blockIdx.x < p.ntiles) tc_issue_tile_loads(a, p, blockIdx.x, stage_h, stage_x, load_bar);
+  if (warp_u == 1 && elect_one_sync() && (int)blockIdx.x < p.ntiles) tc_issue_tile_loads(a, p, blockIdx.x, stage_h, stage_x, nullptr, load_bar);
 
   for (int tile = blockIdx.x; tile < p.ntiles; tile += gridDim.x) {
     const long long g0 = (long long)tile * p.npt;
@@ -389,7 +396,7 @@
         __syncthreads();
         if (ai == 0) STC_TRACE(2);
         if (warp_u == 1 && ai == p.nacc - 1 && tile + (int)gridDim.x < p.ntiles && elect_one_sync())
-          tc_issue_tile_loads(a, p, tile + gridDim.x, stage_h, stage_x, load_bar);
+          tc_issue_tile_loads(a, p, tile + gridDim.x, stage_h, stage_x, nullptr, load_bar);
         if (warp_u == 0 && elect_one_sync()) {
           fence_after_sync();
           const int kleft = p.KBL - j * ATOM_K;
@@ -511,6 +518,11 @@
   if (warp == 0) tmem_dealloc(tmem_base, (uint32_t)p.tmem_cols);
 }
 
+constexpr int FP_THREADS = 512;
+constexpr int FP_EPI_THREADS = 256;
+constexpr int FP_CVT_THREADS = 128;
+__device__ __forceinline__ void fp_epi_sync() { asm volatile("bar.sync 1, 256;" ::: "memory"); }
+
 template <int NG>
 __device__ __forceinline__ void tc_fwd_epilogue_regs(const ConvArgs& a, const TcFwdPlan& p, uint32_t tl, float* Pm,
                                                      const float* Qs, const float* bias_s, const float4 (&hp)[2],
@@ -546,7 +558,7 @@
     tmem_ld8_async(tl + (uint32_t)(p.Npad + 16 * g + cb), sm0[g]);
     tmem_ld8_async(tl + (uint32_t)(16 * g + cb), mn0[g]);
   }
-  __syncthreads();
+  fp_epi_sync();
   tmem_ld_wait();
   float v[NG][8];
 #pragma unroll
@@ -621,8 +633,8 @@
 }
 
 template <int NG>
-__global__ void __launch_bounds__(CV_THREADS, 2)
-tc_conv_fwd_at_kernel(const ConvArgs a, const TcFwdPlan p) {
+__global__ void __launch_bounds__(FP_THREADS, 1)
+tc_conv_fwd_pipe_kernel(const ConvArgs a, const TcFwdPlan p) {
   extern __shared__ __align__(1024) uint8_t smem[];
   if ((smem_u32(smem) & 1023u) != 0u) __trap();
   const int tid = threadIdx.x, warp = tid >> 5, lane = tid & 31;
@@ -634,20 +646,35 @@
   uint8_t* B_lo = B_hi + atomB;
   float* Qs = reinterpret_cast<float*>(smem + p.off_q);
   float* bias_s = reinterpret_cast<float*>(smem + p.off_bias);
-  uint64_t* mma_bar = reinterpret_cast<uint64_t*>(smem + p.off_bar);
-  uint32_t* tmem_slot = reinterpret_cast<uint32_t*>(mma_bar + 1);
+  uint8_t* ring = smem + p.off_sh;
+  uint64_t* full = reinterpret_cast<uint64_t*>(smem + p.off_bar);
+  uint64_t* empty = full + p.nst;
+  uint64_t* a_full = empty + p.nst;
+  uint64_t* a_empty = a_full + 2;
+  uint64_t* acc_full = a_empty + 2;
+  uint64_t* acc_empty = acc_full + 2;
+  uint32_t* tmem_slot = reinterpret_cast<uint32_t*>(acc_empty + 2);
 
   if (tid == 0) {
-    mbar_init(mma_bar, 1);
+    for (int s = 0; s < p.nst; ++s) {
+      mbar_init(full + s, 1);
+      mbar_init(empty + s, FP_EPI_THREADS);
+    }
+    for (int b = 0; b < 2; ++b) {
+      mbar_init(a_full + b, FP_CVT_THREADS);
+      mbar_init(a_empty + b, 1);
+      mbar_init(acc_full + b, 1);
+      mbar_init(acc_empty + b, FP_EPI_THREADS);
+    }
     mbar_fence_init();
   }
-  if (warp == 0) tmem_alloc(tmem_slot, (uint32_t)p.tmem_cols);
-  for (int i = tid; i < C * C; i += CV_THREADS) Qs[i] = a.Q[C * C + i];
-  for (int i = tid; i < Hout; i += CV_THREADS) bias_s[i] = a.bias ? a.bias[i] : 0.f;
+  if (warp == 0) tmem_alloc(tmem_slot, 512u);
+  for (int i = tid; i < C * C; i += FP_THREADS) Qs[i] = a.Q[C * C + i];
+  for (int i = tid; i < Hout; i += FP_THREADS) bias_s[i] = a.bias ? a.bias[i] : 0.f;
   for (int k = 0; k < 2; ++k) {
     uint8_t* bh = B_hi + (size_t)k * 2 * atomB;
     uint8_t* bl = B_lo + (size_t)k * 2 * atomB;
-    for (int it = tid; it < p.Npad * 8; it += CV_THREADS) {
+    for (int it = tid; it < p.Npad * 8; it += FP_THREADS) {
       const int n = it >> 3, qq = it & 7;
       const int c = n / Hout, o = n - c * Hout;
       float v[4];
@@ -666,123 +693,165 @@
   fence_after_sync();
   const int warp_u = uniform_warp_index();
   const uint32_t tmem_base = uniform_u32(*tmem_slot);
-  const uint32_t idesc = make_idesc_tf32(128, p.Npad), idesc2 = make_idesc_tf32(128, 2 * p.Npad);
-  const uint32_t d_main = tmem_base, d_small = tmem_base + (uint32_t)p.Npad;
-  const uint32_t colA = (uint32_t)(2 * p.Npad);
-  const uint64_t dB_hi = make_smem_desc_sw128(smem_u32(B_hi));
-  const int ksteps = p.KBL >> 3;
   const long long total_nodes = (long long)a.B * a.N;
-  const long long R = total_nodes * C;
-
-  const int sp = warp & 3, half = warp >> 2;
-  const int erow = sp * 32 + lane;
-  const int enode = erow / C, ecat = erow - enode * C;
-  const uint32_t tl = tmem_base + ((uint32_t)(sp * 32) << 16);
-  const uint32_t tA = tl + colA + (uint32_t)(half * 32);
-  const bool xvec = p.x_bulk != 0;
-  uint32_t mma_phase = 0;
-  const bool tracing = a.trace != nullptr && blockIdx.x == 0 && tid == 0;
-  int trace_it = 0;
-  for (int tile = blockIdx.x; tile < p.ntiles; tile += gridDim.x) {
-    const long long g0 = (long long)tile * p.npt;
-    const int nodes_valid = (int)min((long long)p.npt, total_nodes - g0);
-    const int rows_valid = nodes_valid * C;
-    const bool valid = erow < rows_valid;
-    const long long gr = g0 * C + erow;
-    STC_TRACE(0);
-    if ((a.opt & OPT_L2_PREFETCH) && warp_u == 1 && tile + (int)gridDim.x < p.ntiles && elect_one_sync())
-      tc_prefetch_tile(a, p, tile + gridDim.x);
-    float4 xv[8];
-#pragma unroll
-    for (int i = 0; i < 8; ++i) xv[i] = make_float4(0.f, 0.f, 0.f, 0.f);
-    if (valid) {
-      const float* hs = (half == 0 ? a.h0 : a.yh) + gr * h;
-#pragma unroll
-      for (int i = 0; i < 4; ++i) xv[i] = *reinterpret_cast<const float4*>(hs + 4 * i);
-      const float* xs;
-      if (half == 0) {
-        const long long g = g0 + enode;
-        const long long b = g / a.N;
-        xs = a.x0 + b * a.x0_bs + ((g - b * a.N) * C + ecat) * Din;
-      } else {
-        xs = a.yx + gr * Din;
-      }
-      if (xvec) {
-#pragma unroll
-        for (int i = 0; i < 4; ++i)
-          if (4 * i < Din) xv[4 + i] = *reinterpret_cast<const float4*>(xs + 4 * i);
-      } else {
-        float e[16];
-#pragma unroll
-        for (int i = 0; i < 16; ++i) e[i] = i < Din ? xs[i] : 0.f;
-#pragma unroll
-        for (int i = 0; i < 4; ++i) xv[4 + i] = make_float4(e[4 * i], e[4 * i + 1], e[4 * i + 2], e[4 * i + 3]);
-      }
-    }
-    STC_TRACE(1);
-#pragma unroll
-    for (int i = 0; i < 4; ++i) {
-      float hi[8], lo[8];
-      split_tf32(xv[2 * i].x, hi[0], lo[0]); split_tf32(xv[2 * i].y, hi[1], lo[1]);
-      split_tf32(xv[2 * i].z, hi[2], lo[2]); split_tf32(xv[2 * i].w, hi[3], lo[3]);
-      split_tf32(xv[2 * i + 1].x, hi[4], lo[4]); split_tf32(xv[2 * i + 1].y, hi[5], lo[5]);
-      split_tf32(xv[2 * i + 1].z, hi[6], lo[6]); split_tf32(xv[2 * i + 1].w, hi[7], lo[7]);
-      tmem_st8(tA + (uint32_t)(8 * i), hi);
-      tmem_st8(tA + 64u + (uint32_t)(8 * i), lo);
-    }
-    tmem_st_wait();
-    STC_TRACE(12);
-    fence_before_sync();
-    STC_TRACE(13);
-    __syncthreads();
-    STC_TRACE(2);
-    STC_TRACE(3);
-    if (warp_u == 0 && elect_one_sync()) {
+  const int nst = p.nst;
+
+  if (warp_u == 1) {
+    if (elect_one_sync()) {
+      const bool tracing = a.trace != nullptr && blockIdx.x == 0;
+      int trace_it = 0;
+      for (int tile = blockIdx.x, i = 0; tile < p.ntiles; tile += gridDim.x, ++i, ++trace_it) {
+        const int s = i % nst;
+        mbar_wait_backoff(empty + s, ((uint32_t)(i / nst) & 1u) ^ 1u, 64);
+        uint8_t* st = ring + (size_t)s * p.stage_bytes;
+        tc_issue_tile_loads(a, p, tile, reinterpret_cast<float*>(st), reinterpret_cast<float*>(st + p.off_sx),
+                            reinterpret_cast<float*>(st + p.off_se), full + s);
+        STC_TRACE(0);
+      }
+    }
+  } else if (warp_u == 0) {
+    const uint32_t idesc = make_idesc_tf32(128, p.Npad), idesc2 = make_idesc_tf32(128, 2 * p.Npad);
+    const uint64_t dB_hi = make_smem_desc_sw128(smem_u32(B_hi));
+    const int ksteps = p.KBL >> 3;
+    for (int tile = blockIdx.x, i = 0; tile < p.ntiles; tile += gridDim.x, ++i) {
+      const int b = i & 1;
+      const uint32_t use = (uint32_t)(i >> 1) & 1u;
+      mbar_wait(a_full + b, use);
+      mbar_wait(acc_empty + b, use ^ 1u);
+      if (elect_one_sync()) {
+        const bool tracing = a.trace != nullptr && blockIdx.x == 0;
+        const int trace_it = i;
+        STC_TRACE(3);
+        fence_after_sync();
+        const uint32_t d_main = tmem_base + (uint32_t)(2 * p.Npad * b), d_small = d_main + (uint32_t)p.Npad;
+        const uint32_t colA = 256u + 128u * (uint32_t)b;
+        uint32_t acc = 0u;
+#pragma unroll
+        for (int ai = 0; ai < 2; ++ai) {
+          const uint64_t bo = (uint64_t)(((uint32_t)ai * 2u * atomB) >> 4);
+          for (int ks = 0; ks < ksteps; ++ks) {
+            const uint64_t ko = (uint64_t)(ks * 2);
+            const uint32_t ah = tmem_base + colA + (uint32_t)(ai * 32 + ks * 8), al = ah + 64u;
+            mma_tf32_atmem(d_main, ah, dB_hi + bo + ko, idesc2, acc);
+            mma_tf32_atmem(d_small, al, dB_hi + bo + ko, idesc, 1u);
+            acc = 1u;
+          }
+        }
+        mma_commit(acc_full + b);
+        mma_commit(a_empty + b);
+        STC_TRACE(4);
+      }
+      __syncwarp();
+    }
+  } else if (warp_u >= 4 && warp_u < 8) {
+    const int erow = (warp_u & 3) * 32 + lane;
+    const int enode = erow / C, ecat = erow - enode * C;
+    const uint32_t tA0 = tmem_base + ((uint32_t)((warp_u & 3) * 32) << 16) + 256u;
+    const bool xvec = p.x_bulk != 0;
+    const bool tracing = a.trace != nullptr && blockIdx.x == 0 && erow == 0;
+    for (int tile = blockIdx.x, i = 0; tile < p.ntiles; tile += gridDim.x, ++i) {
+      const int trace_it = i;
+      const int s = i % nst, b = i & 1;
+      const long long g0 = (long long)tile * p.npt;
+      const int rows_valid = (int)min((long long)p.npt, total_nodes - g0) * C;
+      const bool valid = erow < rows_valid;
+      const long long gr = g0 * C + erow;
+      const uint8_t* st = ring + (size_t)s * p.stage_bytes;
+      mbar_wait(full + s, (uint32_t)(i / nst) & 1u);
+      STC_TRACE(1);
+      float4 xv[2][8];
+#pragma unroll
+      for (int k = 0; k < 2; ++k) {
+#pragma unroll
+        for (int j = 0; j < 8; ++j) xv[k][j] = make_float4(0.f, 0.f, 0.f, 0.f);
+        if (valid) {
+          const float* hs = reinterpret_cast<const float*>(st) + (k * 128 + erow) * h;
+#pragma unroll
+          for (int j = 0; j < 4; ++j) xv[k][j] = *reinterpret_cast<const float4*>(hs + 4 * j);
+          if (xvec) {
+            const float* xs = reinterpret_cast<const float*>(st + p.off_sx) + (k * 128 + erow) * Din;
+#pragma unroll
+            for (int j = 0; j < 4; ++j)
+              if (4 * j < Din) xv[k][4 + j] = *reinterpret_cast<const float4*>(xs + 4 * j);
+          } else {
+            const float* xs;
+            if (k == 0) {
+              const long long g = g0 + enode;
+              const long long bb = g / a.N;
+              xs = a.x0 + bb * a.x0_bs + ((g - bb * a.N) * C + ecat) * Din;
+            } else {
+              xs = a.yx + gr * Din;
+            }
+            float e[16];
+#pragma unroll
+            for (int j = 0; j < 16; ++j) e[j] = j < Din ? xs[j] : 0.f;
+#pragma unroll
+            for (int j = 0; j < 4; ++j) xv[k][4 + j] = make_float4(e[4 * j], e[4 * j + 1], e[4 * j + 2], e[4 * j + 3]);
+          }
+        }
+      }
+      mbar_wait(a_empty + b, ((uint32_t)(i >> 1) & 1u) ^ 1u);
       fence_after_sync();
-      uint32_t acc = 0u;
-#pragma unroll
-      for (int ai = 0; ai < 2; ++ai) {
-        const uint64_t bo = (uint64_t)(((uint32_t)ai * 2u * atomB) >> 4);
-        for (int ks = 0; ks < ksteps; ++ks) {
-          const uint64_t ko = (uint64_t)(ks * 2);
-          const uint32_t ah = tmem_base + colA + (uint32_t)(ai * 32 + ks * 8), al = ah + 64u;
-          mma_tf32_atmem(d_main, ah, dB_hi + bo + ko, idesc2, acc);
-          mma_tf32_atmem(d_small, al, dB_hi + bo + ko, idesc, 1u);
-          acc = 1u;
+      const uint32_t tA = tA0 + 128u * (uint32_t)b;
+#pragma unroll
+      for (int k = 0; k < 2; ++k) {
+#pragma unroll
+        for (int j = 0; j < 4; ++j) {
+          float hi[8], lo[8];
+          split_tf32(xv[k][2 * j].x, hi[0], lo[0]); split_tf32(xv[k][2 * j].y, hi[1], lo[1]);
+          split_tf32(xv[k][2 * j].z, hi[2], lo[2]); split_tf32(xv[k][2 * j].w, hi[3], lo[3]);
+          split_tf32(xv[k][2 * j + 1].x, hi[4], lo[4]); split_tf32(xv[k][2 * j + 1].y, hi[5], lo[5]);
+          split_tf32(xv[k][2 * j + 1].z, hi[6], lo[6]); split_tf32(xv[k][2 * j + 1].w, hi[7], lo[7]);
+          tmem_st8(tA + (uint32_t)(32 * k + 8 * j), hi);
+          tmem_st8(tA + 64u + (uint32_t)(32 * k + 8 * j), lo);
         }
       }
-      STC_TRACE(8);
-      STC_TRACE(10);
-      mma_commit(mma_bar);
-      STC_TRACE(9);
-      STC_TRACE(11);
-    }
-    float4 hp[2], uu[2];
-    hp[0] = hp[1] = uu[0] = uu[1] = make_float4(0.f, 0.f, 0.f, 0.f);
-    if (valid) {
-      const float* hsrc = a.Hprev + gr * h + half * 8;
-      hp[0] = *reinterpret_cast<const float4*>(hsrc);
-      hp[1] = *reinterpret_cast<const float4*>(hsrc + 4);
+      tmem_st_wait();
+      fence_before_sync();
+      mbar_arrive(a_full + b);
+      STC_TRACE(2);
+    }
+  } else if (warp_u >= 8) {
+    const int sp = warp_u & 3, half = (warp_u - 8) >> 2;
+    const int erow = sp * 32 + lane;
+    const int enode = erow / C, ecat = erow - enode * C;
+    const uint32_t tl = tmem_base + ((uint32_t)(sp * 32) << 16);
+    const bool tracing = a.trace != nullptr && blockIdx.x == 0 && erow == 0 && half == 0;
+    for (int tile = blockIdx.x, i = 0; tile < p.ntiles; tile += gridDim.x, ++i) {
+      const int trace_it = i;
+      const int s = i % nst, b = i & 1;
+      const long long g0 = (long long)tile * p.npt;
+      const int rows_valid = (int)min((long long)p.npt, total_nodes - g0) * C;
+      const bool valid = erow < rows_valid;
+      const long long gr = g0 * C + erow;
+      mbar_wait(acc_full + b, (uint32_t)(i >> 1) & 1u);
+      mbar_wait(full + s, (uint32_t)(i / nst) & 1u);
+      fence_after_sync();
+      STC_TRACE(5);
+      const float* se = reinterpret_cast<const float*>(ring + (size_t)s * p.stage_bytes + p.off_se);
+      float4 hp[2], uu[2];
+      hp[0] = *reinterpret_cast<const float4*>(se + erow * h + half * 8);
+      hp[1] = *reinterpret_cast<const float4*>(se + erow * h + half * 8 + 4);
+      uu[0] = uu[1] = make_float4(0.f, 0.f, 0.f, 0.f);
       if (a.phase != 0) {
-        const float* usrc = a.u + gr * h + half * 8;
-        uu[0] = *reinterpret_cast<const float4*>(usrc);
-        uu[1] = *reinterpret_cast<const float4*>(usrc + 4);
-      }
-    }
-    STC_TRACE(4);
-    mbar_wait(mma_bar, mma_phase);
-    mma_phase ^= 1u;
+        uu[0] = *reinterpret_cast<const float4*>(se + 128 * h + erow * h + half * 8);
+        uu[1] = *reinterpret_cast<const float4*>(se + 128 * h + erow * h + half * 8 + 4);
+      }
+      tc_fwd_epilogue_regs<NG>(a, p, tl + (uint32_t)(2 * p.Npad * b), Pm + (size_t)b * 128 * p.PS, Qs, bias_s, hp, uu,
+                               erow, enode, ecat, half, valid, gr);
+      fence_before_sync();
+      mbar_arrive(acc_empty + b);
+      fence_async_smem();
+      mbar_arrive(empty + s);
+      STC_TRACE(6);
+    }
+  }
+  fence_before_sync();
+  __syncthreads();
+  if (warp == 0) {
     fence_after_sync();
-    STC_TRACE(5);
-    STC_TRACE(6);
-    tc_fwd_epilogue_regs<NG>(a, p, tl, Pm, Qs, bias_s, hp, uu, erow, enode, ecat, half, valid, gr);
-    STC_TRACE(7);
-    ++trace_it;
-    fence_before_sync();
-    __syncthreads();
-  }
-  __syncthreads();
-  if (warp == 0) tmem_dealloc(tmem_base, (uint32_t)p.tmem_cols);
+    tmem_dealloc(tmem_base, 512u);
+  }
 }
 
 static bool tc_disabled() {
@@ -865,30 +934,50 @@
   int ng = 0;
   if (a.Kc == 2 && p.nmain == 1 && (a.Hout == 16 || a.Hout == 32) && !(a.opt & OPT_GENERIC_EPILOGUE)) ng = a.Hout / 16;
   auto kern = ng == 2 ? tc_conv_fwd_kernel<2> : (ng == 1 ? tc_conv_fwd_kernel<1> : tc_conv_fwd_kernel<0>);
-  const bool at = ng != 0 && a.Ks == 2 && a.h == 16 && p.KB == 1 && !(a.opt & OPT_SMEM_A);
+  bool at = ng != 0 && a.Ks == 2 && a.h == 16 && p.KB == 1 && !(a.opt & OPT_SMEM_A);
+  TcFwdPlan pp = p;
   if (at) {
-    kern = ng == 2 ? tc_conv_fwd_at_kernel<2> : tc_conv_fwd_at_kernel<1>;
     size_t q = 0;
-    p.off_a = (uint32_t)q; q += round_up((size_t)128 * p.PS * sizeof(float), 1024);
-    p.off_b = (uint32_t)q; q += 2 * (size_t)2 * atomB;
-    p.off_q = (uint32_t)q; q += round_up((size_t)a.C * a.C * sizeof(float), 16);
-    p.off_bias = (uint32_t)q; q += round_up((size_t)a.Hout * sizeof(float), 16);
-    p.off_bar = (uint32_t)q; q += 32;
-    p.smem_bytes = (uint32_t)q;
-    p.tmem_cols = 256;
-  }
-  if (!at && smem_over) return declined("shared memory");
-  STC_TRY(set_smem(kern, p.smem_bytes));
-  int ctas_per_sm = (int)((228 * 1024) / (p.smem_bytes + 1024));
-  if (ctas_per_sm < 1) ctas_per_sm = 1;
-  if (ctas_per_sm > 2) ctas_per_sm = 2;
-  if (ctas_per_sm * p.tmem_cols > 512) ctas_per_sm = 512 / p.tmem_cols;
-  int grid = device_sm_count() * ctas_per_sm;
+    pp.off_a = (uint32_t)q; q += 2 * round_up((size_t)128 * p.PS * sizeof(float), 1024);
+    pp.off_b = (uint32_t)q; q += 2 * (size_t)2 * atomB;
+    pp.off_q = (uint32_t)q; q += round_up((size_t)a.C * a.C * sizeof(float), 16);
+    pp.off_bias = (uint32_t)q; q += round_up((size_t)a.Hout * sizeof(float), 16);
+    pp.off_bar = (uint32_t)q;
+    size_t sb = 0;
+    sb += (size_t)a.Ks * 128 * a.h * sizeof(float);
+    pp.off_sx = (uint32_t)sb; sb += p.x_bulk ? round_up((size_t)a.Ks * 128 * a.Din * sizeof(float), 16) : 0;
+    pp.off_se = (uint32_t)sb; sb += (size_t)2 * 128 * a.h * sizeof(float);
+    pp.stage_bytes = (uint32_t)round_up(sb, 128);
+    const size_t cap = 227 * 1024;
+    pp.nst = 4;
+    while (pp.nst > 2 && q + (size_t)(2 * pp.nst + 9) * 8 + 127 + (size_t)pp.nst * pp.stage_bytes > cap) --pp.nst;
+    q += round_up((size_t)(2 * pp.nst + 9) * 8, 128);
+    pp.off_sh = (uint32_t)q; q += (size_t)pp.nst * pp.stage_bytes;
+    pp.smem_bytes = (uint32_t)q;
+    pp.tmem_cols = 512;
+    at = pp.smem_bytes <= cap;
+  }
+  int threads = CV_THREADS, grid;
+  if (at) {
+    p = pp;
+    kern = ng == 2 ? tc_conv_fwd_pipe_kernel<2> : tc_conv_fwd_pipe_kernel<1>;
+    threads = FP_THREADS;
+    STC_TRY(set_smem(kern, p.smem_bytes));
+    grid = device_sm_count();
+  } else {
+    if (smem_over) return declined("shared memory");
+    STC_TRY(set_smem(kern, p.smem_bytes));
+    int ctas_per_sm = (int)((228 * 1024) / (p.smem_bytes + 1024));
+    if (ctas_per_sm < 1) ctas_per_sm = 1;
+    if (ctas_per_sm > 2) ctas_per_sm = 2;
+    if (ctas_per_sm * p.tmem_cols > 512) ctas_per_sm = 512 / p.tmem_cols;
+    grid = device_sm_count() * ctas_per_sm;
+  }
   if (grid > p.ntiles) grid = p.ntiles;
   const double R = (double)total_nodes * a.C;
   ScopedKernelTimer _t(KK_TC_CONV_FWD, st,
                        4.0 * R * (a.Ks * L + (a.phase == 0 ? 3 * a.h : 4 * a.h)) + 4.0 * P * L * a.Hout);
-  kern<<<grid, CV_THREADS, p.smem_bytes, st>>>(a, p);
+  kern<<<grid, threads, p.smem_bytes, st>>>(a, p);
   STC_LAUNCH_OK("tc_conv_fwd_kernel");
   *handled = true;
   return STC_OK;
diff --git a/stc_gnn_b200/csrc/stc_conv_tc_bwd.cu b/stc_gnn_b200/csrc/stc_conv_tc_bwd.cu
--- a/stc_gnn_b200/csrc/stc_conv_tc_bwd.cu
+++ b/stc_gnn_b200/csrc/stc_conv_tc_bwd.cu
@@ -18,7 +18,9 @@
   int DP;
   int PW;
   int x_vec;
+  int nst;
   uint32_t off_a, off_b, off_ds, off_dh, off_ps, off_q, off_acc, off_bar, smem_bytes;
+  uint32_t stage_bytes;
 };
 
 struct DxIn {
@@ -90,7 +92,7 @@
   }
 }
 
-template <bool FAST, bool AT>
+template <bool FAST>
 __global__ void __launch_bounds__(CV_THREADS, 2)
 tc_conv_bwd_dx_kernel(const ConvArgs a, const TcDxPlan p) {
   extern __shared__ __align__(1024) uint8_t smem[];
@@ -103,8 +105,7 @@
   uint8_t* A_hi = smem + p.off_a;
   uint8_t* A_lo = A_hi + atomA;
   uint8_t* B_hi = smem + p.off_b;
-  uint8_t* B_lo = B_hi + (AT ? (size_t)atomB : (size_t)p.KA * atomB);
-  const size_t bstride = AT ? 2 * (size_t)atomB : (size_t)atomB;
+  uint8_t* B_lo = B_hi + (size_t)p.KA * atomB;
   float* Dsm = reinterpret_cast<float*>(smem + p.off_ds);
   float* Dh = reinterpret_cast<float*>(smem + p.off_dh);
   float* Psm = reinterpret_cast<float*>(smem + p.off_ps);
@@ -125,8 +126,8 @@
     dQacc[i] = 0.f;
   }
   for (int ja = 0; ja < p.KA; ++ja) {
-    uint8_t* bh = B_hi + (size_t)ja * bstride;
-    uint8_t* bl = B_lo + (size_t)ja * bstride;
+    uint8_t* bh = B_hi + (size_t)ja * atomB;
+    uint8_t* bl = B_lo + (size_t)ja * atomB;
     for (int it = tid; it < p.Npad * 8; it += CV_THREADS) {
       const int n = it >> 3, qq = it & 7;
       const int k = n / p.KBL, kb = n - k * p.KBL;
@@ -147,7 +148,7 @@
   fence_after_sync();
   const int warp_u = uniform_warp_index();
   const uint32_t tmem_base = uniform_u32(*tmem_slot);
-  const uint32_t idesc = make_idesc_tf32(128, p.Npad), idesc2 = make_idesc_tf32(128, 2 * p.Npad);
+  const uint32_t idesc = make_idesc_tf32(128, p.Npad);
   const uint32_t d_small = tmem_base + (uint32_t)(p.nmain * p.Npad);
   const uint64_t dA_hi = make_smem_desc_sw128(smem_u32(A_hi)), dA_lo = make_smem_desc_sw128(smem_u32(A_lo));
   const uint64_t dB_hi = make_smem_desc_sw128(smem_u32(B_hi)), dB_lo = make_smem_desc_sw128(smem_u32(B_lo));
@@ -230,149 +231,67 @@
       for (int row = db_grp; row < rows_valid; row += db_groups) s += Dsm[row * DP + db_col];
       db_acc += s;
     }
-    if constexpr (AT) {
-      const int cw = Hout >> 1;
-      const int cbase = cw * half;
-      const int enode = erow / C, ecat = erow - enode * C;
-      const float* qrow = Qs + ecat * C;
-      const uint32_t tA = tl + (uint32_t)(2 * p.Npad);
-      const bool two = cw == 16;
-      float dm[16];
-#pragma unroll
-      for (int i = 0; i < 16; ++i) dm[i] = 0.f;
-      {
-        const float* sp = Dsm + (enode * C) * DP + cbase;
-#pragma unroll 5
-        for (int d = 0; d < C; ++d) {
-          const float w = qrow[d];
-          const float4 x0 = *reinterpret_cast<const float4*>(sp + d * DP);
-          const float4 x1 = *reinterpret_cast<const float4*>(sp + d * DP + 4);
-          dm[0] = fmaf(w, x0.x, dm[0]); dm[1] = fmaf(w, x0.y, dm[1]); dm[2] = fmaf(w, x0.z, dm[2]); dm[3] = fmaf(w, x0.w, dm[3]);
-          dm[4] = fmaf(w, x1.x, dm[4]); dm[5] = fmaf(w, x1.y, dm[5]); dm[6] = fmaf(w, x1.z, dm[6]); dm[7] = fmaf(w, x1.w, dm[7]);
-          if (two) {
-            const float4 x2 = *reinterpret_cast<const float4*>(sp + d * DP + 8);
-            const float4 x3 = *reinterpret_cast<const float4*>(sp + d * DP + 12);
-            dm[8] = fmaf(w, x2.x, dm[8]); dm[9] = fmaf(w, x2.y, dm[9]); dm[10] = fmaf(w, x2.z, dm[10]); dm[11] = fmaf(w, x2.w, dm[11]);
-            dm[12] = fmaf(w, x3.x, dm[12]); dm[13] = fmaf(w, x3.y, dm[13]); dm[14] = fmaf(w, x3.z, dm[14]); dm[15] = fmaf(w, x3.w, dm[15]);
-          }
-        }
-      }
-      if (erow < rows_valid) {
-        float* dp = a.dpre + (row0 + erow) * p.Kdd + Hout + cbase;
-        *reinterpret_cast<float4*>(dp) = make_float4(dm[0], dm[1], dm[2], dm[3]);
-        *reinterpret_cast<float4*>(dp + 4) = make_float4(dm[4], dm[5], dm[6], dm[7]);
-        if (two) {
-          *reinterpret_cast<float4*>(dp + 8) = make_float4(dm[8], dm[9], dm[10], dm[11]);
-          *reinterpret_cast<float4*>(dp + 12) = make_float4(dm[12], dm[13], dm[14], dm[15]);
-        }
-      }
-#pragma unroll
-      for (int part = 0; part < 2; ++part) {
-        if (part * 8 < cw) {
-          const int col = cbase + part * 8;
-          float hi[8], lo[8];
-          {
-            const float4 x0 = *reinterpret_cast<const float4*>(Dsm + erow * DP + col);
-            const float4 x1 = *reinterpret_cast<const float4*>(Dsm + erow * DP + col + 4);
-            split_tf32(x0.x, hi[0], lo[0]); split_tf32(x0.y, hi[1], lo[1]); split_tf32(x0.z, hi[2], lo[2]); split_tf32(x0.w, hi[3], lo[3]);
-            split_tf32(x1.x, hi[4], lo[4]); split_tf32(x1.y, hi[5], lo[5]); split_tf32(x1.z, hi[6], lo[6]); split_tf32(x1.w, hi[7], lo[7]);
-          }
-          tmem_st8(tA + (uint32_t)col, hi);
-          tmem_st8(tA + 64u + (uint32_t)col, lo);
-#pragma unroll
-          for (int i = 0; i < 8; ++i) split_tf32(dm[part * 8 + i], hi[i], lo[i]);
-          tmem_st8(tA + (uint32_t)(Hout + col), hi);
-          tmem_st8(tA + 64u + (uint32_t)(Hout + col), lo);
-        }
-      }
-      tmem_st_wait();
-      STC_TRACE(12);
-      fence_before_sync();
-      STC_TRACE(13);
+    bool acc_small = false;
+    for (int ja = 0; ja < p.KA; ++ja) {
+      const int kk = ja * ATOM_K + q * 4;
+      const int c = kk / Hout, o0 = kk - c * Hout;
+      float4 vv[4];
+#pragma unroll
+      for (int i = 0; i < 4; ++i) {
+        float4 v = make_float4(0.f, 0.f, 0.f, 0.f);
+        if (kk < p.Kdd) {
+          if (c == 0) {
+            v = *reinterpret_cast<const float4*>(Dsm + (r0 + 32 * i) * DP + o0);
+          } else {
+            const float* Qc = Qs + (size_t)(c - 1) * C * C + rcat[i] * C;
+            const float* sp = Dsm + rnode[i] * C * DP + o0;
+            for (int d = 0; d < C; ++d) {
+              const float w = Qc[d];
+              const float4 x = *reinterpret_cast<const float4*>(sp + d * DP);
+              v.x = fmaf(w, x.x, v.x); v.y = fmaf(w, x.y, v.y); v.z = fmaf(w, x.z, v.z); v.w = fmaf(w, x.w, v.w);
+            }
+            if (r0 + 32 * i < rows_valid)
+              *reinterpret_cast<float4*>(a.dpre + (row0 + r0 + 32 * i) * p.Kdd + kk) = v;
+          }
+        }
+        vv[i] = v;
+      }
+      if (mma_pending) {
+        mbar_wait(mma_bar, mma_phase);
+        mma_phase ^= 1u;
+        mma_pending = false;
+      }
+#pragma unroll
+      for (int i = 0; i < 4; ++i) store_split4(A_hi, A_lo, aoff[i], vv[i]);
+      if (ja == 0) STC_TRACE(12);
+      fence_async_smem();
+      if (ja == 0) STC_TRACE(13);
       __syncthreads();
-      STC_TRACE(2);
+      if (ja == 0) STC_TRACE(2);
       if (warp_u == 0 && elect_one_sync()) {
         fence_after_sync();
-        const uint32_t a0 = tmem_base + (uint32_t)(2 * p.Npad);
-        uint32_t acc = 0u;
-        const int nks = p.Kdd >> 3;
-        for (int ks = 0; ks < nks; ++ks) {
-          const uint64_t bo = (uint64_t)((((uint32_t)(ks >> 2)) * 2u * atomB) >> 4) + (uint64_t)((ks & 3) * 2);
-          const uint32_t ah = a0 + (uint32_t)(ks * 8), al = ah + 64u;
-          mma_tf32_atmem(tmem_base, ah, dB_hi + bo, idesc2, acc);
-          mma_tf32_atmem(d_small, al, dB_hi + bo, idesc, 1u);
-          acc = 1u;
-        }
-        STC_TRACE(8);
-        STC_TRACE(10);
+        const int kleft = p.Kdd - ja * ATOM_K;
+        const int ksteps = kleft >= ATOM_K ? 4 : (kleft + 7) / 8;
+        const uint64_t bo = (uint64_t)(((uint32_t)ja * atomB) >> 4);
+        const uint32_t d_main = tmem_base + (uint32_t)((ja / DX_APM) * p.Npad);
+        uint32_t acc_main = (ja % DX_APM) != 0 ? 1u : 0u;
+#pragma unroll 4
+        for (int ks = 0; ks < ksteps; ++ks) {
+          const uint64_t ko = (uint64_t)(ks * 2);
+          mma_tf32(d_small, dA_lo + ko, dB_hi + bo + ko, idesc, acc_small ? 1u : 0u);
+          mma_tf32(d_small, dA_hi + ko, dB_lo + bo + ko, idesc, 1u);
+          mma_tf32(d_main, dA_hi + ko, dB_hi + bo + ko, idesc, acc_main);
+          acc_main = 1u;
+          acc_small = true;
+        }
+        if (ja == 0) STC_TRACE(8);
+        if (ja == p.KA - 1) STC_TRACE(10);
         mma_commit(mma_bar);
-        STC_TRACE(9);
-        STC_TRACE(11);
-      }
+        if (ja == 0) STC_TRACE(9);
+        if (ja == p.KA - 1) STC_TRACE(11);
+      }
+      acc_small = true;
       mma_pending = true;
-    } else {
-      bool acc_small = false;
-      for (int ja = 0; ja < p.KA; ++ja) {
-        const int kk = ja * ATOM_K + q * 4;
-        const int c = kk / Hout, o0 = kk - c * Hout;
-        float4 vv[4];
-  #pragma unroll
-        for (int i = 0; i < 4; ++i) {
-          float4 v = make_float4(0.f, 0.f, 0.f, 0.f);
-          if (kk < p.Kdd) {
-            if (c == 0) {
-              v = *reinterpret_cast<const float4*>(Dsm + (r0 + 32 * i) * DP + o0);
-            } else {
-              const float* Qc = Qs + (size_t)(c - 1) * C * C + rcat[i] * C;
-              const float* sp = Dsm + rnode[i] * C * DP + o0;
-              for (int d = 0; d < C; ++d) {
-                const float w = Qc[d];
-                const float4 x = *reinterpret_cast<const float4*>(sp + d * DP);
-                v.x = fmaf(w, x.x, v.x); v.y = fmaf(w, x.y, v.y); v.z = fmaf(w, x.z, v.z); v.w = fmaf(w, x.w, v.w);
-              }
-              if (r0 + 32 * i < rows_valid)
-                *reinterpret_cast<float4*>(a.dpre + (row0 + r0 + 32 * i) * p.Kdd + kk) = v;
-            }
-          }
-          vv[i] = v;
-        }
-        if (mma_pending) {
-          mbar_wait(mma_bar, mma_phase);
-          mma_phase ^= 1u;
-          mma_pending = false;
-        }
-  #pragma unroll
-        for (int i = 0; i < 4; ++i) store_split4(A_hi, A_lo, aoff[i], vv[i]);
-        if (ja == 0) STC_TRACE(12);
-        fence_async_smem();
-        if (ja == 0) STC_TRACE(13);
-        __syncthreads();
-        if (ja == 0) STC_TRACE(2);
-        if (warp_u == 0 && elect_one_sync()) {
-          fence_after_sync();
-          const int kleft = p.Kdd - ja * ATOM_K;
-          const int ksteps = kleft >= ATOM_K ? 4 : (kleft + 7) / 8;
-          const uint64_t bo = (uint64_t)(((uint32_t)ja * atomB) >> 4);
-          const uint32_t d_main = tmem_base + (uint32_t)((ja / DX_APM) * p.Npad);
-          uint32_t acc_main = (ja % DX_APM) != 0 ? 1u : 0u;
-  #pragma unroll 4
-          for (int ks = 0; ks < ksteps; ++ks) {
-            const uint64_t ko = (uint64_t)(ks * 2);
-            mma_tf32(d_small, dA_lo + ko, dB_hi + bo + ko, idesc, acc_small ? 1u : 0u);
-            mma_tf32(d_small, dA_hi + ko, dB_lo + bo + ko, idesc, 1u);
-            mma_tf32(d_main, dA_hi + ko, dB_hi + bo + ko, idesc, acc_main);
-            acc_main = 1u;
-            acc_small = true;
-          }
-          if (ja == 0) STC_TRACE(8);
-          if (ja == p.KA - 1) STC_TRACE(10);
-          mma_commit(mma_bar);
-          if (ja == 0) STC_TRACE(9);
-          if (ja == p.KA - 1) STC_TRACE(11);
-        }
-        acc_small = true;
-        mma_pending = true;
-      }
     }
     STC_TRACE(3);
     float4 xprev[4];
@@ -618,6 +537,459 @@
   if (want_dQ)
     for (int i = tid; i < (a.Kc - 1) * C * C; i += CV_THREADS) atomicAdd(&a.dQ[C * C + i], dQacc[i]);
   if (warp == 0) tmem_dealloc(tmem_base, (uint32_t)p.tmem_cols);
+}
+
+constexpr int DP_THREADS = 512;
+constexpr int DP_CVT_THREADS = 256;
+constexpr int DP_EPI_THREADS = 128;
+__device__ __forceinline__ void dp_cvt_sync() { asm volatile("bar.sync 1, 256;" ::: "memory"); }
+
+__global__ void __launch_bounds__(DP_THREADS, 1)
+tc_conv_bwd_dx_pipe_kernel(const ConvArgs a, const TcDxPlan p) {
+  extern __shared__ __align__(1024) uint8_t smem[];
+  if ((smem_u32(smem) & 1023u) != 0u) __trap();
+  const int tid = threadIdx.x, warp = tid >> 5, lane = tid & 31;
+  const int C = a.C, L = a.Din + a.h, Din = a.Din, Hout = a.Hout, DP = p.DP;
+  constexpr int h = 16;
+  const bool want_dQ = a.dQ != nullptr;
+  const uint32_t atomB = (uint32_t)p.Npad * ATOM_ROW_BYTES;
+  uint8_t* B_hi = smem + p.off_b;
+  uint8_t* B_lo = B_hi + atomB;
+  float* Dsm = reinterpret_cast<float*>(smem + p.off_ds);
+  float* Qs = reinterpret_cast<float*>(smem + p.off_q);
+  float* dQacc = reinterpret_cast<float*>(smem + p.off_acc);
+  uint8_t* ring = smem + p.off_a;
+  uint64_t* full = reinterpret_cast<uint64_t*>(smem + p.off_bar);
+  uint64_t* empty = full + p.nst;
+  uint64_t* a_full = empty + p.nst;
+  uint64_t* a_empty = a_full + 2;
+  uint64_t* acc_full = a_empty + 2;
+  uint64_t* acc_empty = acc_full + 2;
+  uint32_t* tmem_slot = reinterpret_cast<uint32_t*>(acc_empty + 2);
+
+  if (tid == 0) {
+    for (int s = 0; s < p.nst; ++s) {
+      mbar_init(full + s, 1);
+      mbar_init(empty + s, DP_CVT_THREADS + DP_EPI_THREADS);
+    }
+    for (int b = 0; b < 2; ++b) {
+      mbar_init(a_full + b, DP_CVT_THREADS);
+      mbar_init(a_empty + b, 1);
+      mbar_init(acc_full + b, 1);
+      mbar_init(acc_empty + b, DP_EPI_THREADS);
+    }
+    mbar_fence_init();
+  }
+  if (warp == 0) tmem_alloc(tmem_slot, 512u);
+  for (int i = tid; i < C * C; i += DP_THREADS) {
+    Qs[i] = a.Q[C * C + i];
+    dQacc[i] = 0.f;
+  }
+  for (int ja = 0; ja < p.KA; ++ja) {
+    uint8_t* bh = B_hi + (size_t)ja * 2 * atomB;
+    uint8_t* bl = B_lo + (size_t)ja * 2 * atomB;
+    for (int it = tid; it < p.Npad * 8; it += DP_THREADS) {
+      const int n = it >> 3, qq = it & 7;
+      const int k = n / p.KBL, kb = n - k * p.KBL;
+      const int l = kb < h ? Din + kb : (kb - h < Din ? kb - h : -1);
+      float v[4];
+#pragma unroll
+      for (int i = 0; i < 4; ++i) {
+        const int kk = ja * ATOM_K + qq * 4 + i;
+        const int c = kk / Hout, o = kk - c * Hout;
+        v[i] = (n < p.N1 && l >= 0 && kk < p.Kdd) ? a.W[((size_t)(k * a.Kc + c) * L + l) * Hout + o] : 0.f;
+      }
+      store_split4(bh, bl, atom_chunk_offset(n, qq), make_float4(v[0], v[1], v[2], v[3]));
+    }
+  }
+  fence_async_smem();
+  fence_before_sync();
+  __syncthreads();
+  fence_after_sync();
+  const int warp_u = uniform_warp_index();
+  const uint32_t tmem_base = uniform_u32(*tmem_slot);
+  const long long total_nodes = (long long)a.B * a.N;
+  const int nst = p.nst;
+  const int nin = a.phase == 0 ? 6 : 3;
+  constexpr int DQ_C = 5;
+  const int dq_chunks = Hout >> 2;
+  const bool dq_fast = want_dQ && C <= DQ_C && p.npt * dq_chunks <= DP_CVT_THREADS;
+  float dq[DQ_C * DQ_C];
+#pragma unroll
+  for (int i = 0; i < DQ_C * DQ_C; ++i) dq[i] = 0.f;
+  float4 dbs0 = make_float4(0.f, 0.f, 0.f, 0.f), dbs1 = dbs0;
+
+  if (warp_u == 1) {
+    if (elect_one_sync()) {
+      const bool tracing = a.trace != nullptr && blockIdx.x == 0;
+      int trace_it = 0;
+      for (int tile = blockIdx.x, i = 0; tile < p.ntiles; tile += gridDim.x, ++i, ++trace_it) {
+        const int s = i % nst;
+        mbar_wait_backoff(empty + s, ((uint32_t)(i / nst) & 1u) ^ 1u, 64);
+        float* st = reinterpret_cast<float*>(ring + (size_t)s * p.stage_bytes);
+        const long long g0 = (long long)tile * p.npt;
+        const int rows_valid = (int)min((long long)p.npt, total_nodes - g0) * C;
+        const long long o = g0 * C * h;
+        const uint32_t hb = (uint32_t)(rows_valid * h * 4), pb = want_dQ ? (uint32_t)(rows_valid * p.PW * 4) : 0u;
+        mbar_arrive_expect_tx(full + s, (uint32_t)nin * hb + pb);
+        bulk_g2s(st, a.dHn + o, hb, full + s);
+        bulk_g2s(st + 128 * h, a.u + o, hb, full + s);
+        bulk_g2s(st + 2 * 128 * h, a.c + o, hb, full + s);
+        if (a.phase == 0) {
+          bulk_g2s(st + 3 * 128 * h, a.Hprev + o, hb, full + s);
+          bulk_g2s(st + 4 * 128 * h, a.r + o, hb, full + s);
+          bulk_g2s(st + 5 * 128 * h, a.drH + o, hb, full + s);
+        }
+        if (want_dQ) bulk_g2s(reinterpret_cast<uint8_t*>(st) + p.off_ps, a.Psave + g0 * C * p.PW, pb, full + s);
+        STC_TRACE(0);
+      }
+    }
+  } else if (warp_u == 0) {
+    const uint32_t idesc = make_idesc_tf32(128, p.Npad), idesc2 = make_idesc_tf32(128, 2 * p.Npad);
+    const uint64_t dB_hi = make_smem_desc_sw128(smem_u32(B_hi));
+    const int nks = p.Kdd >> 3;
+    for (int tile = blockIdx.x, i = 0; tile < p.ntiles; tile += gridDim.x, ++i) {
+      const int b = i & 1;
+      const uint32_t use = (uint32_t)(i >> 1) & 1u;
+      mbar_wait(a_full + b, use);
+      mbar_wait(acc_empty + b, use ^ 1u);
+      if (elect_one_sync()) {
+        const bool tracing = a.trace != nullptr && blockIdx.x == 0;
+        const int trace_it = i;
+        STC_TRACE(3);
+        fence_after_sync();
+        const uint32_t d_main = tmem_base + (uint32_t)(2 * p.Npad * b), d_small = d_main + (uint32_t)p.Npad;
+        const uint32_t a0 = tmem_base + 256u + 128u * (uint32_t)b;
+        uint32_t acc = 0u;
+        for (int ks = 0; ks < nks; ++ks) {
+          const uint64_t bo = (uint64_t)((((uint32_t)(ks >> 2)) * 2u * atomB) >> 4) + (uint64_t)((ks & 3) * 2);
+          const uint32_t ah = a0 + (uint32_t)(ks * 8), al = ah + 64u;
+          mma_tf32_atmem(d_main, ah, dB_hi + bo, idesc2, acc);
+          mma_tf32_atmem(d_small, al, dB_hi + bo, idesc, 1u);
+          acc = 1u;
+        }
+        mma_commit(acc_full + b);
+        mma_commit(a_empty + b);
+        STC_TRACE(4);
+      }
+      __syncwarp();
+    }
+  } else if (warp_u >= 8) {
+    const int ctid = tid - 8 * 32;
+    const int sp = warp_u & 3, half = (warp_u - 8) >> 2;
+    const int erow = sp * 32 + lane;
+    const int enode = erow / C, ecat = erow - enode * C;
+    const uint32_t tA0 = tmem_base + ((uint32_t)(sp * 32) << 16) + 256u;
+    const int dq_node = ctid / dq_chunks, dq_oc = (ctid - dq_node * dq_chunks) << 2;
+    const bool tracing = a.trace != nullptr && blockIdx.x == 0 && ctid == 0;
+    for (int tile = blockIdx.x, i = 0; tile < p.ntiles; tile += gridDim.x, ++i) {
+      const int trace_it = i;
+      const int s = i % nst, b = i & 1;
+      const long long g0 = (long long)tile * p.npt;
+      const int nodes_valid = (int)min((long long)p.npt, total_nodes - g0);
+      const int rows_valid = nodes_valid * C;
+      const long long row0 = g0 * C;
+      const float* st = reinterpret_cast<const float*>(ring + (size_t)s * p.stage_bytes);
+      const float* Psm = reinterpret_cast<const float*>(ring + (size_t)s * p.stage_bytes + p.off_ps);
+      float* Dh = reinterpret_cast<float*>(ring + (size_t)s * p.stage_bytes + p.off_dh);
+      float* Ds = Dsm + (size_t)b * 128 * DP;
+      mbar_wait(full + s, (uint32_t)(i / nst) & 1u);
+      STC_TRACE(1);
+      constexpr int cpr = h >> 2;
+      for (int it = ctid; it < 128 * cpr; it += DP_CVT_THREADS) {
+        const int row = it / cpr, j = (it - row * cpr) << 2;
+        float4 g0v = make_float4(0.f, 0.f, 0.f, 0.f), g1v = g0v, dir = g0v;
+        const bool live = row < rows_valid;
+        if (live) {
+          const int so = row * h + j;
+          DxIn in;
+          in.dhn = *reinterpret_cast<const float4*>(st + so);
+          in.uu = *reinterpret_cast<const float4*>(st + 128 * h + so);
+          in.cc = *reinterpret_cast<const float4*>(st + 2 * 128 * h + so);
+          if (a.phase == 0) {
+            in.hp = *reinterpret_cast<const float4*>(st + 3 * 128 * h + so);
+            in.rr = *reinterpret_cast<const float4*>(st + 4 * 128 * h + so);
+            in.drh = *reinterpret_cast<const float4*>(st + 5 * 128 * h + so);
+          }
+          dx_adjoint(a, in, g0v, g1v, dir);
+          *reinterpret_cast<float4*>(a.dpre + (row0 + row) * p.Kdd + j) = g0v;
+          if (a.phase == 0) *reinterpret_cast<float4*>(a.dpre + (row0 + row) * p.Kdd + h + j) = g1v;
+        }
+        dbs0.x += g0v.x; dbs0.y += g0v.y; dbs0.z += g0v.z; dbs0.w += g0v.w;
+        dbs1.x += g1v.x; dbs1.y += g1v.y; dbs1.z += g1v.z; dbs1.w += g1v.w;
+        *reinterpret_cast<float4*>(Ds + row * DP + j) = g0v;
+        if (a.phase == 0) {
+          *reinterpret_cast<float4*>(Ds + row * DP + h + j) = g1v;
+          *reinterpret_cast<float4*>(Dh + row * h + j) = dir;
+        }
+      }
+      dp_cvt_sync();
+      const int cw = Hout >> 1;
+      const int cbase = cw * half;
+      const float* qrow = Qs + ecat * C;
+      const bool two = cw == 16;
+      float dm[16];
+#pragma unroll
+      for (int k = 0; k < 16; ++k) dm[k] = 0.f;
+      {
+        const float* spp = Ds + (enode * C) * DP + cbase;
+#pragma unroll 5
+        for (int d = 0; d < C; ++d) {
+          const float w = qrow[d];
+          const float4 x0 = *reinterpret_cast<const float4*>(spp + d * DP);
+          const float4 x1 = *reinterpret_cast<const float4*>(spp + d * DP + 4);
+          dm[0] = fmaf(w, x0.x, dm[0]); dm[1] = fmaf(w, x0.y, dm[1]); dm[2] = fmaf(w, x0.z, dm[2]); dm[3] = fmaf(w, x0.w, dm[3]);
+          dm[4] = fmaf(w, x1.x, dm[4]); dm[5] = fmaf(w, x1.y, dm[5]); dm[6] = fmaf(w, x1.z, dm[6]); dm[7] = fmaf(w, x1.w, dm[7]);
+          if (two) {
+            const float4 x2 = *reinterpret_cast<const float4*>(spp + d * DP + 8);
+            const float4 x3 = *reinterpret_cast<const float4*>(spp + d * DP + 12);
+            dm[8] = fmaf(w, x2.x, dm[8]); dm[9] = fmaf(w, x2.y, dm[9]); dm[10] = fmaf(w, x2.z, dm[10]); dm[11] = fmaf(w, x2.w, dm[11]);
+            dm[12] = fmaf(w, x3.x, dm[12]); dm[13] = fmaf(w, x3.y, dm[13]); dm[14] = fmaf(w, x3.z, dm[14]); dm[15] = fmaf(w, x3.w, dm[15]);
+          }
+        }
+      }
+      if (erow < rows_valid) {
+        float* dp = a.dpre + (row0 + erow) * p.Kdd + Hout + cbase;
+        *reinterpret_cast<float4*>(dp) = make_float4(dm[0], dm[1], dm[2], dm[3]);
+        *reinterpret_cast<float4*>(dp + 4) = make_float4(dm[4], dm[5], dm[6], dm[7]);
+        if (two) {
+          *reinterpret_cast<float4*>(dp + 8) = make_float4(dm[8], dm[9], dm[10], dm[11]);
+          *reinterpret_cast<float4*>(dp + 12) = make_float4(dm[12], dm[13], dm[14], dm[15]);
+        }
+      }
+      mbar_wait(a_empty + b, ((uint32_t)(i >> 1) & 1u) ^ 1u);
+      fence_after_sync();
+      const uint32_t tA = tA0 + 128u * (uint32_t)b;
+#pragma unroll
+      for (int part = 0; part < 2; ++part) {
+        if (part * 8 < cw) {
+          const int col = cbase + part * 8;
+          float hi[8], lo[8];
+          {
+            const float4 x0 = *reinterpret_cast<const float4*>(Ds + erow * DP + col);
+            const float4 x1 = *reinterpret_cast<const float4*>(Ds + erow * DP + col + 4);
+            split_tf32(x0.x, hi[0], lo[0]); split_tf32(x0.y, hi[1], lo[1]); split_tf32(x0.z, hi[2], lo[2]); split_tf32(x0.w, hi[3], lo[3]);
+            split_tf32(x1.x, hi[4], lo[4]); split_tf32(x1.y, hi[5], lo[5]); split_tf32(x1.z, hi[6], lo[6]); split_tf32(x1.w, hi[7], lo[7]);
+          }
+          tmem_st8(tA + (uint32_t)col, hi);
+          tmem_st8(tA + 64u + (uint32_t)col, lo);
+#pragma unroll
+          for (int k = 0; k < 8; ++k) split_tf32(dm[part * 8 + k], hi[k], lo[k]);
+          tmem_st8(tA + (uint32_t)(Hout + col), hi);
+          tmem_st8(tA + 64u + (uint32_t)(Hout + col), lo);
+        }
+      }
+      tmem_st_wait();
+      fence_before_sync();
+      mbar_arrive(a_full + b);
+      STC_TRACE(2);
+      if (want_dQ) {
+        const int npairs = C * C;
+        const int groups = DP_CVT_THREADS / npairs;
+        if (dq_fast) {
+          if (dq_node < nodes_valid) {
+            float4 pv[DQ_C], dv[DQ_C];
+#pragma unroll
+            for (int k = 0; k < DQ_C; ++k) {
+              const int ci = k < C ? k : 0;
+              pv[k] = *reinterpret_cast<const float4*>(Psm + (dq_node * C + ci) * p.PW + dq_oc);
+              dv[k] = *reinterpret_cast<const float4*>(Ds + (dq_node * C + ci) * DP + dq_oc);
+            }
+#pragma unroll
+            for (int cp = 0; cp < DQ_C; ++cp)
+#pragma unroll
+              for (int d = 0; d < DQ_C; ++d) {
+                float sacc = dq[cp * DQ_C + d];
+                sacc = fmaf(pv[cp].x, dv[d].x, sacc); sacc = fmaf(pv[cp].y, dv[d].y, sacc);
+                sacc = fmaf(pv[cp].z, dv[d].z, sacc); sacc = fmaf(pv[cp].w, dv[d].w, sacc);
+                dq[cp * DQ_C + d] = sacc;
+              }
+          }
+        } else if (groups >= 1) {
+          const int pr = ctid % npairs, grp = ctid / npairs;
+          if (grp < groups) {
+            const int cp = pr / C, d = pr - cp * C;
+            float sacc = 0.f;
+            for (int node = grp; node < nodes_valid; node += groups) {
+              const float* pp = Psm + (node * C + cp) * p.PW;
+              const float* dd = Ds + (node * C + d) * DP;
+              for (int o = 0; o < Hout; o += 4) {
+                const float4 x = *reinterpret_cast<const float4*>(pp + o);
+                const float4 y = *reinterpret_cast<const float4*>(dd + o);
+                sacc = fmaf(x.x, y.x, sacc); sacc = fmaf(x.y, y.y, sacc); sacc = fmaf(x.z, y.z, sacc); sacc = fmaf(x.w, y.w, sacc);
+              }
+            }
+            atomicAdd(&dQacc[pr], sacc);
+          }
+        } else {
+          for (int pr = ctid; pr < npairs; pr += DP_CVT_THREADS) {
+            const int cp = pr / C, d = pr - cp * C;
+            float sacc = 0.f;
+            for (int node = 0; node < nodes_valid; ++node) {
+              const float* pp = Psm + (node * C + cp) * p.PW;
+              const float* dd = Ds + (node * C + d) * DP;
+              for (int o = 0; o < Hout; ++o) sacc = fmaf(pp[o], dd[o], sacc);
+            }
+            dQacc[pr] += sacc;
+          }
+        }
+      }
+      fence_async_smem();
+      mbar_arrive(empty + s);
+      STC_TRACE(7);
+    }
+  } else if (warp_u >= 4) {
+    const int sp = warp_u & 3;
+    const int erow = sp * 32 + lane;
+    const uint32_t tl = tmem_base + ((uint32_t)(sp * 32) << 16);
+    const bool tracing = a.trace != nullptr && blockIdx.x == 0 && erow == 0;
+    const bool xpre = a.accum_x && p.x_vec;
+    for (int tile = blockIdx.x, i = 0; tile < p.ntiles; tile += gridDim.x, ++i) {
+      const int trace_it = i;
+      const int s = i % nst, b = i & 1;
+      const long long g0 = (long long)tile * p.npt;
+      const int rows_valid = (int)min((long long)p.npt, total_nodes - g0) * C;
+      const bool valid = erow < rows_valid;
+      const long long gr = g0 * C + erow;
+      float4 xprev[2][4];
+#pragma unroll
+      for (int k = 0; k < 2; ++k) {
+#pragma unroll
+        for (int j = 0; j < 4; ++j) xprev[k][j] = make_float4(0.f, 0.f, 0.f, 0.f);
+        const float* dbase_pf = (k == 0 ? a.dYx0 : a.dYx);
+        if (xpre && valid && dbase_pf != nullptr) {
+          const float* src = dbase_pf + gr * Din;
+#pragma unroll
+          for (int j = 0; j < 4; ++j)
+            if (4 * j < Din) xprev[k][j] = *reinterpret_cast<const float4*>(src + 4 * j);
+        }
+      }
+      mbar_wait(acc_full + b, (uint32_t)(i >> 1) & 1u);
+      mbar_wait(a_full + b, (uint32_t)(i >> 1) & 1u);
+      fence_after_sync();
+      STC_TRACE(5);
+      const uint32_t ts = tl + (uint32_t)(2 * p.Npad * b);
+      const float* Dh = reinterpret_cast<const float*>(ring + (size_t)s * p.stage_bytes + p.off_dh);
+#pragma unroll
+      for (int k = 0; k < 2; ++k) {
+        const uint32_t nb = (uint32_t)(k * p.KBL);
+        {
+          uint32_t sm[16], mn[16];
+          tmem_ld16_async(ts + (uint32_t)p.Npad + nb, sm);
+          tmem_ld16_async(ts + nb, mn);
+          tmem_ld_wait();
+          tmem_ld_pin16(sm); tmem_ld_pin16(mn);
+          if (valid) {
+            float v[16];
+#pragma unroll
+            for (int j = 0; j < 16; ++j) v[j] = __uint_as_float(sm[j]) + __uint_as_float(mn[j]);
+            if (k == 0 && a.phase == 0) {
+#pragma unroll
+              for (int j = 0; j < 16; j += 4) {
+                const float4 d = *reinterpret_cast<const float4*>(Dh + erow * 16 + j);
+                v[j] += d.x; v[j + 1] += d.y; v[j + 2] += d.z; v[j + 3] += d.w;
+              }
+            }
+            float* dst = (k == 0 ? a.dYh0 : a.dYh) + gr * 16;
+#pragma unroll
+            for (int j = 0; j < 16; j += 4) *reinterpret_cast<float4*>(dst + j) = make_float4(v[j], v[j + 1], v[j + 2], v[j + 3]);
+          }
+        }
+        float* dbase = (k == 0 ? a.dYx0 : a.dYx);
+        {
+          uint32_t sm[16], mn[16];
+          if (p.Dp == 16) {
+            tmem_ld16_async(ts + (uint32_t)p.Npad + nb + 16u, sm);
+            tmem_ld16_async(ts + nb + 16u, mn);
+            tmem_ld_wait();
+            tmem_ld_pin16(sm); tmem_ld_pin16(mn);
+          } else {
+            uint32_t s8[8], m8[8];
+            tmem_ld8_async(ts + (uint32_t)p.Npad + nb + 16u, s8);
+            tmem_ld8_async(ts + nb + 16u, m8);
+            tmem_ld_wait();
+            tmem_ld_pin8(s8); tmem_ld_pin8(m8);
+#pragma unroll
+            for (int j = 0; j < 8; ++j) { sm[j] = s8[j]; mn[j] = m8[j]; sm[j + 8] = 0u; mn[j + 8] = 0u; }
+          }
+          if (valid && dbase != nullptr) {
+            float* dst = dbase + gr * Din;
+            if (p.x_vec) {
+              float4 o[4];
+#pragma unroll
+              for (int j = 0; j < 4; ++j)
+                o[j] = make_float4(__uint_as_float(sm[4 * j]) + __uint_as_float(mn[4 * j]),
+                                   __uint_as_float(sm[4 * j + 1]) + __uint_as_float(mn[4 * j + 1]),
+                                   __uint_as_float(sm[4 * j + 2]) + __uint_as_float(mn[4 * j + 2]),
+                                   __uint_as_float(sm[4 * j + 3]) + __uint_as_float(mn[4 * j + 3]));
+              if (a.accum_x) {
+#pragma unroll
+                for (int j = 0; j < 4; ++j)
+                  if (4 * j < Din) { o[j].x += xprev[k][j].x; o[j].y += xprev[k][j].y; o[j].z += xprev[k][j].z; o[j].w += xprev[k][j].w; }
+              }
+#pragma unroll
+              for (int j = 0; j < 4; ++j)
+                if (4 * j < Din) *reinterpret_cast<float4*>(dst + 4 * j) = o[j];
+            } else {
+#pragma unroll
+              for (int j = 0; j < 16; ++j)
+                if (j < Din) {
+                  const float vi = __uint_as_float(sm[j]) + __uint_as_float(mn[j]);
+                  dst[j] = a.accum_x ? dst[j] + vi : vi;
+                }
+            }
+          }
+        }
+      }
+      fence_before_sync();
+      mbar_arrive(acc_empty + b);
+      mbar_arrive(empty + s);
+      STC_TRACE(6);
+    }
+  }
+  fence_before_sync();
+  __syncthreads();
+  const bool cvt = warp_u >= 8;
+  if (a.dbias) {
+    for (int i = tid; i < Hout; i += DP_THREADS) Dsm[i] = 0.f;
+    __syncthreads();
+    if (cvt) {
+      constexpr int cprw = h >> 2;
+      float v[8] = {dbs0.x, dbs0.y, dbs0.z, dbs0.w, dbs1.x, dbs1.y, dbs1.z, dbs1.w};
+      for (int off = cprw; off < 32; off <<= 1) {
+#pragma unroll
+        for (int i = 0; i < 8; ++i) v[i] += __shfl_xor_sync(0xffffffffu, v[i], off);
+      }
+      if (lane < cprw) {
+        const int j = (lane % cprw) << 2;
+        atomicAdd(&Dsm[j + 0], v[0]); atomicAdd(&Dsm[j + 1], v[1]); atomicAdd(&Dsm[j + 2], v[2]); atomicAdd(&Dsm[j + 3], v[3]);
+        if (a.phase == 0) {
+          atomicAdd(&Dsm[h + j + 0], v[4]); atomicAdd(&Dsm[h + j + 1], v[5]);
+          atomicAdd(&Dsm[h + j + 2], v[6]); atomicAdd(&Dsm[h + j + 3], v[7]);
+        }
+      }
+    }
+    __syncthreads();
+    for (int i = tid; i < Hout; i += DP_THREADS) atomicAdd(&a.dbias[i], Dsm[i]);
+  }
+  if (dq_fast && cvt) {
+#pragma unroll
+    for (int cp = 0; cp < DQ_C; ++cp)
+#pragma unroll
+      for (int d = 0; d < DQ_C; ++d) {
+        float sacc = dq[cp * DQ_C + d];
+#pragma unroll
+        for (int off = 16; off >= 1; off >>= 1) sacc += __shfl_xor_sync(0xffffffffu, sacc, off);
+        if (lane == 0 && cp < C && d < C) atomicAdd(&dQacc[cp * C + d], sacc);
+      }
+  }
+  __syncthreads();
+  if (want_dQ)
+    for (int i = tid; i < C * C; i += DP_THREADS) atomicAdd(&a.dQ[C * C + i], dQacc[i]);
+  if (warp == 0) {
+    fence_after_sync();
+    tmem_dealloc(tmem_base, 512u);
+  }
 }
 
 static bool aligned16b(const void* p) { return (reinterpret_cast<uintptr_t>(p) & 15) == 0; }
@@ -663,22 +1035,50 @@
     return STC_ERR_UNSUPPORTED;
   }
   const bool fast = a.Ks == 2 && a.h == 16 && a.Din <= 16 && p.nmain == 1 && !(a.opt & OPT_GENERIC_EPILOGUE);
-  const bool at = fast && a.Kc == 2 && p.Kdd <= 64 && (a.Hout == 16 || a.Hout == 32) && !(a.opt & OPT_SMEM_A);
-  auto kern = at ? tc_conv_bwd_dx_kernel<true, true>
-                 : (fast ? tc_conv_bwd_dx_kernel<true, false> : tc_conv_bwd_dx_kernel<false, false>);
-  if (at) p.tmem_cols = 256;
-  STC_TRY(set_smem(kern, p.smem_bytes));
-  int ctas_per_sm = (int)((228 * 1024) / (p.smem_bytes + 1024));
-  if (ctas_per_sm < 1) ctas_per_sm = 1;
-  if (ctas_per_sm > 2) ctas_per_sm = 2;
-  if (ctas_per_sm * p.tmem_cols > 512) ctas_per_sm = 512 / p.tmem_cols;
-  int grid = device_sm_count() * ctas_per_sm;
+  bool at = fast && a.Kc == 2 && p.Kdd <= 64 && (a.Hout == 16 || a.Hout == 32) && !(a.opt & OPT_SMEM_A);
+  TcDxPlan pp = p;
+  if (at) {
+    size_t q = 0;
+    pp.off_b = (uint32_t)q; q += 2 * (size_t)p.KA * atomB;
+    pp.off_ds = (uint32_t)q; q += 2 * (size_t)128 * p.DP * sizeof(float);
+    pp.off_q = (uint32_t)q; q += round_up((size_t)a.C * a.C * sizeof(float), 16);
+    pp.off_acc = (uint32_t)q; q += round_up((size_t)a.C * a.C * sizeof(float), 16);
+    pp.off_bar = (uint32_t)q;
+    size_t sb = (size_t)(a.phase == 0 ? 6 : 3) * 128 * a.h * sizeof(float);
+    pp.off_ps = (uint32_t)sb; sb += (size_t)128 * p.PW * sizeof(float);
+    pp.off_dh = (uint32_t)sb; sb += a.phase == 0 ? (size_t)128 * a.h * sizeof(float) : 0;
+    pp.stage_bytes = (uint32_t)round_up(sb, 128);
+    const size_t cap = 227 * 1024;
+    pp.nst = 4;
+    while (pp.nst > 2 && q + (size_t)(2 * pp.nst + 9) * 8 + 127 + (size_t)pp.nst * pp.stage_bytes > cap) --pp.nst;
+    q += round_up((size_t)(2 * pp.nst + 9) * 8, 128);
+    pp.off_a = (uint32_t)q; q += (size_t)pp.nst * pp.stage_bytes;
+    pp.smem_bytes = (uint32_t)q;
+    pp.tmem_cols = 512;
+    at = pp.smem_bytes <= cap;
+  }
+  auto kern = fast ? tc_conv_bwd_dx_kernel<true> : tc_conv_bwd_dx_kernel<false>;
+  int threads = CV_THREADS, grid;
+  if (at) {
+    p = pp;
+    kern = tc_conv_bwd_dx_pipe_kernel;
+    threads = DP_THREADS;
+    STC_TRY(set_smem(kern, p.smem_bytes));
+    grid = device_sm_count();
+  } else {
+    STC_TRY(set_smem(kern, p.smem_bytes));
+    int ctas_per_sm = (int)((228 * 1024) / (p.smem_bytes + 1024));
+    if (ctas_per_sm < 1) ctas_per_sm = 1;
+    if (ctas_per_sm > 2) ctas_per_sm = 2;
+    if (ctas_per_sm * p.tmem_cols > 512) ctas_per_sm = 512 / p.tmem_cols;
+    grid = device_sm_count() * ctas_per_sm;
+  }
   if (grid > p.ntiles) grid = p.ntiles;
   const double R = (double)total_nodes * a.C;
   ScopedKernelTimer _t(KK_TC_CONV_BWD_DX, st,
                        4.0 * R * ((a.phase == 0 ? 6 * a.h + a.Ks * a.Din : 3 * a.h) + a.Hout + a.Ks * L +
                                   ((a.dQ && a.Kc > 1) ? p.PW : 0)) + 4.0 * a.Ks * a.Kc * L * a.Hout);
-  kern<<<grid, CV_THREADS, p.smem_bytes, st>>>(a, p);
+  kern<<<grid, threads, p.smem_bytes, st>>>(a, p);
   STC_LAUNCH_OK("tc_conv_bwd_dx_kernel");
   *handled = true;
   return STC_OK;
```

Result: faster. 63920, median of 6 (+3.5%).
